# bacpop/ska.rust

Hardware: AMD Instinct MI355X
Metric: genomes/sec ska build+align, 1 000x5 Mbp k=31; bit-exact vs CPU (higher is better)
Workload: dtype u64

## Files before the change

include/skx.h:

```cpp
#ifndef SKX_H
#define SKX_H
#include <stddef.h>
#include <stdint.h>

#ifdef __cplusplus
extern "C" {
#endif

#define SKX_OK        0
#define SKX_EINVAL    1
#define SKX_EIO       2
#define SKX_ENODEV    3
#define SKX_ENOMEM    4
#define SKX_EEMPTY    5
#define SKX_EUNSUP    6
#define SKX_EFORMAT   7

enum { SKX_QUAL_NOFILTER = 0, SKX_QUAL_MIDDLE = 1, SKX_QUAL_STRICT = 2 };
enum { SKX_FILTER_NONE = 0, SKX_FILTER_NO_CONST = 1, SKX_FILTER_NO_AMBIG = 2, SKX_FILTER_NO_AMBIG_OR_CONST = 3 };

typedef struct {
    uint16_t min_count;
    uint8_t  min_qual;
    int32_t  qual_filter;
// ... 96 lines not shown
                               int64_t *constant, uint64_t *rows_used, skx_select_info *info);
int  skx_array_distance_select_prefiltered(skx_array *a, int64_t constant, int filt_ambig, const skx_select_spec *spec, skx_dist_pair **pairs,
                                           uint64_t *n_pairs, skx_select_info *info);
typedef struct { double max_snps, max_mismatches; int32_t band_rows; } skx_mst_spec;
typedef struct { uint64_t bands, band_rows, count_buffer_bytes, candidates, edges, components, rounds; } skx_mst_info;
int  skx_array_distance_mst(skx_array *a, double min_freq, int filt_ambig, const skx_mst_spec *spec, skx_dist_pair **pairs, uint64_t *n_pairs,
                            int64_t *constant, uint64_t *rows_used, skx_mst_info *info);
int  skx_array_distance_mst_prefiltered(skx_array *a, int64_t constant, int filt_ambig, const skx_mst_spec *spec, skx_dist_pair **pairs,
                                        uint64_t *n_pairs, skx_mst_info *info);
int  skx_array_distance_planes(skx_array *a, int filt_ambig, const void **planes, uint64_t *words_per_row, int *n_planes);
int  skx_planes_distance(skx_ctx *ctx, const void *planes, int n_samples, uint64_t words_per_row, int filt_ambig, double constant,
                         int i_lo, int i_hi, skx_dist *out);
void skx_free(void *p);

typedef struct skx_comm skx_comm;
#define SKX_COMM_ID_BYTES 128
int  skx_comm_unique_id(uint8_t id[SKX_COMM_ID_BYTES]);
int  skx_comm_create(skx_ctx *ctx, int rank, int world, const uint8_t id[SKX_COMM_ID_BYTES], skx_comm **out);
int  skx_comm_create_local(skx_ctx *ctx, int rank, int world, const char *dir, skx_comm **out);
void skx_comm_destroy(skx_comm *c);
int  skx_comm_rank(const skx_comm *c);
int  skx_comm_world(const skx_comm *c);
uint64_t skx_comm_bytes_received(const skx_comm *c);
int  skx_comm_transport(const skx_comm *c, int *rccl_ranks, int *rccl_device, int *ctx_device);
int  skx_comm_barrier(skx_comm *c);
int  skx_comm_allgather(skx_comm *c, const void *send, void *recv, uint64_t bytes, int on_device);
int  skx_comm_allreduce_u32(skx_comm *c, uint32_t *buf, uint64_t n, int on_device);
int  skx_comm_gather_root(skx_comm *c, const void *send, const uint64_t *sizes, void *recv);
int  skx_shard_range(uint64_t n_items, int rank, int world, uint64_t *lo, uint64_t *hi);
int  skx_pair_bands(int n_samples, int world, int align, int *lo_hi);
int  skx_keyset_allgather(skx_comm *c, skx_keyset *local, skx_keyset **rows);
int  skx_array_reduce_stats(skx_comm *c, skx_array *a, uint64_t total_samples);
int  skx_array_distance_sharded(skx_comm *c, skx_array *a, int filt_ambig, double constant, skx_dist *out, uint64_t n_out);


int  skx_array_merge(skx_ctx *ctx, skx_array *const *arrays, int n_arrays, skx_array **out);
int  skx_array_delete_samples(skx_array *a, const char *const *names, int n_names);
typedef struct { uint64_t rows_present, removed, silent, sites; } skx_subset_info;
int  skx_array_subset_filtered(skx_array *a, const int *samples, int n_samples, const skx_filter_spec *f,
                               skx_array **out, skx_subset_info *info);
int  skx_array_weed(skx_array *a, skx_keyset *weed, int reverse, uint64_t *removed);
int  skx_keyset_from_fasta(skx_ctx *ctx, const char *path, int k, int rc, skx_keyset **out);
int  skx_cov_histogram(skx_ctx *ctx, const char *fastq_fwd, const char *fastq_rev, int k, int rc, uint32_t *hist);

int  skx_array_map(skx_array *a, const char *reference_fasta, int ambig_mask, int repeat_mask, int format, int threads, char **buf, uint64_t *len);
int  skx_skf_peek_k(const char *path);
skx_ctx *skx_array_ctx(const skx_array *a);
void skx_set_last_error(const char *msg);

typedef struct skx_lo_graph skx_lo_graph;
typedef struct {
    int32_t  k, words_per_node;
    uint64_t n_samples, colour_words;
    uint64_t n_nodes, n_edges, n_entries;
    uint64_t n_colours;
    uint64_t n_kmers;
} skx_lo_info;
int  skx_array_lo_graph(skx_array *a, skx_lo_graph **out);
int  skx_lo_graph_info(const skx_lo_graph *g, skx_lo_info *info);
int  skx_lo_graph_export(const skx_lo_graph *g, uint64_t *nodes, uint64_t *offsets, uint64_t *neighbours, uint64_t *entries, uint64_t *exits);
int  skx_lo_gather(skx_lo_graph *g, const uint64_t *kmers, uint64_t n, uint64_t *colours, uint8_t *found);
void skx_lo_graph_free(skx_lo_graph *g);

typedef struct { uint32_t a, b; double len_a, len_b; } skx_nj_join;
int  skx_dist_nj(skx_ctx *ctx, const skx_dist *d, int n_samples, skx_nj_join *joins);
int  skx_matrix_nj(skx_ctx *ctx, const double *m, int n, skx_nj_join *joins);

typedef struct {
    double  cluster_snps, cluster_mismatches;
    int32_t band_rows;
} skx_banded_spec;
typedef struct { uint64_t bands, band_rows, count_buffer_bytes, edges, clusters; } skx_banded_info;
int  skx_array_distance_banded(skx_array *a, double min_freq, int filt_ambig, const skx_banded_spec *spec,
                               uint32_t *labels, skx_nj_join *joins, int64_t *constant, uint64_t *rows_used, skx_banded_info *info);
int  skx_array_distance_banded_prefiltered(skx_array *a, int64_t constant, int filt_ambig, const skx_banded_spec *spec,
                                           uint32_t *labels, skx_nj_join *joins, skx_banded_info *info);

int  skx_phases_json(char **buf, uint64_t *len, int reset);
void skx_phase_add(const char *name, double seconds);

typedef struct { double hist, scatter, dedupe, key_union, assemble, filter, compact, distance, append_probe, append, pieces_stats, pieces_rows; } skx_timings;
int  skx_ctx_timings(skx_ctx *ctx, skx_timings *t, int reset);
const char *skx_ctx_merge_path(skx_ctx *ctx);

#ifdef __cplusplus
}
#endif
#endif
```

ska.rust_amd/csrc/skx_api.cpp:

```cpp
#include "skx_internal.h"
#include "../../include/skx_host.h"
#include <algorithm>
#include <atomic>
#include <chrono>
#include <cmath>
#include <cstdarg>
#include <cstddef>
#include <cstdio>
#include <cstring>
#include <map>
#include <memory>
#include <mutex>
#include <numeric>
#include <optional>
#include <unordered_map>
#include <thread>
#include <cerrno>
#include <fcntl.h>
#include <sys/mman.h>
#include <sys/stat.h>
#include <unistd.h>

using namespace skx;

// ... 129 lines not shown
}

int skx::check_k(int k)
{
    if (k < 5 || k > 63 || (k & 1) == 0) { set_error("Invalid k-mer length"); return SKX_EINVAL; }
    return SKX_OK;
}

skx::Preallocator::Preallocator(int fd_, off_t base_) : fd(fd_), base(base_)
{
    th = std::thread([this]() {
        constexpr uint64_t STEP = 256ull << 20;
        std::unique_lock<std::mutex> lk(mu);
        for (;;) {
            cv.wait(lk, [this] { return stop || done < target; });
            if (stop && done >= target) return;
            const uint64_t o = done, n = std::min(STEP, target - done);
            lk.unlock();
            if (posix_fallocate(fd, base + (off_t)o, (off_t)n) != 0) failed.store(true, std::memory_order_release);
            lk.lock();
            done = o + n;
            cv.notify_all();
        }
    });
}
skx::Preallocator::~Preallocator() { { std::lock_guard<std::mutex> lk(mu); stop = true; target = done; } cv.notify_all(); if (th.joinable()) th.join(); }
void skx::Preallocator::raise(uint64_t bytes) { { std::lock_guard<std::mutex> lk(mu); if (bytes > target) target = bytes; } cv.notify_all(); }
void skx::Preallocator::finish(uint64_t bytes)
{
    std::unique_lock<std::mutex> lk(mu);
    if (bytes > target) target = bytes;
    cv.notify_all();
    cv.wait(lk, [&] { return done >= bytes; });
}
bool skx::mappable_output_fd(int fd, off_t *pos)
{
    struct stat sb;
    if (fstat(fd, &sb) != 0 || !S_ISREG(sb.st_mode)) return false;
    const int fl = fcntl(fd, F_GETFL);
    if (fl < 0 || (fl & O_APPEND) || (fl & O_ACCMODE) != O_RDWR) return false;
    *pos = lseek(fd, 0, SEEK_CUR);
    return *pos >= 0;
}
extern "C" int skx_ctx_expect_output(skx_ctx *ctx, int fd)
{
    if (!ctx) return SKX_EINVAL;
    off_t pos;
    ctx->expect_fd = (fd >= 0 && mappable_output_fd(fd, &pos)) ? fd : -1;
    return SKX_OK;
}

extern "C" int skx_ctx_create(int device, skx_ctx **out)
{
    return skx_guarded([&]() -> int {
    if (!out) { set_error("null out"); return SKX_EINVAL; }
    int ndev = 0;
    hipError_t e = hipGetDeviceCount(&ndev);
    if (e != hipSuccess || ndev <= 0) { set_error("no HIP device available (%s); the engine has no CPU path", e == hipSuccess ? "count 0" : hipGetErrorString(e)); return SKX_ENODEV; }
    if (device < 0 || device >= ndev) { set_error("device %d out of range (%d devices)", device, ndev); return SKX_EINVAL; }
    SKX_HIP(hipSetDevice(device));
    skx_ctx *c = new skx_ctx();
    c->device = device;
    if (hipStreamCreateWithFlags(&c->stream, hipStreamNonBlocking) != hipSuccess ||
        hipEventCreate(&c->ev[0]) != hipSuccess || hipEventCreate(&c->ev[1]) != hipSuccess || hipEventCreate(&c->ev[2]) != hipSuccess ||
        hipEventCreate(&c->ev[3]) != hipSuccess) {
        delete c; set_error("cannot create HIP stream/events"); return SKX_ENODEV;
    }
    *out = c;
    return SKX_OK;
    });
}
extern "C" void skx_ctx_destroy(skx_ctx *c)
{
    if (!c) return;
    if (c->stream) { (void)hipStreamSynchronize(c->stream); (void)hipStreamDestroy(c->stream); }
    for (auto &e : c->ev) if (e) (void)hipEventDestroy(e);
    skx::dev_trim();
    delete c;
}
extern "C" int skx_ctx_sync(skx_ctx *c) { SKX_HIP(hipSetDevice(c->device)); SKX_HIP(hipStreamSynchronize(c->stream)); return SKX_OK; }
extern "C" void *skx_ctx_stream(skx_ctx *c) { return (void *)c->stream; }
uint64_t skx::next_object_id() { static std::atomic<uint64_t> n{0}; return ++n; }
extern "C" const char *skx_ctx_merge_path(skx_ctx *c) { return c ? c->merge_path.c_str() : ""; }
extern "C" int skx_ctx_timings(skx_ctx *c, skx_timings *t, int reset)
{
    return skx_guarded([&]() -> int {
    if (t) *t = c->tm;
    if (reset) c->tm = skx_timings{};
    return SKX_OK;
    });
}

namespace {
struct KernelTimer {
    skx_ctx *c; double *slot;
    KernelTimer(skx_ctx *c_, double *s) : c(c_), slot(s) { if (c->timing) (void)hipEventRecord(c->ev[2], c->stream); }
    ~KernelTimer()
    {
        if (!c->timing) return;
        (void)hipEventRecord(c->ev[3], c->stream);
        (void)hipEventSynchronize(c->ev[3]);
        float ms = 0; if (hipEventElapsedTime(&ms, c->ev[2], c->ev[3]) == hipSuccess) *slot += ms;
    }
};
int ilog2_ceil(uint64_t x) { int l = 0; while ((1ull << l) < x) l++; return l; }
constexpr uint32_t LDS_TABLE_MAX = 18000;
constexpr uint32_t LDS_SORT_MAX = 6144;
constexpr uint32_t LDS_SORT_MAX_WIDE = 4096;
}

extern "C" void skx_dictset_free(skx_dictset *d) { delete d; }
extern "C" int skx_dictset_nsamples(const skx_dictset *d) { return d->n; }
extern "C" int skx_dictset_key_bits(const skx_dictset *d) { return d->key_bits; }

int skx::reads_words_to_dictset(skx_ctx *ctx, std::vector<DevBuf<uint64_t>> &wl, std::vector<DevBuf<uint64_t>> &wh2, const std::vector<uint64_t> &cnt,
                                int k, int rc, skx_dictset **out)
{
    const int n = (int)wl.size();
    hipStream_t st = ctx->stream;
    const bool wide_r = k > 31;
    const int wpk_r = wide_r ? 2 : 1, kbits = 2 * (k - 1);
    uint64_t maxn = 0;
    for (auto c : cnt) maxn = std::max(maxn, c);
    const uint64_t per = wide_r ? 2500 : 3500, lds_max = wide_r ? LDS_SORT_MAX_WIDE : LDS_SORT_MAX;
    int logB = std::min({ilog2_ceil((maxn + per - 1) / per), kbits, MAX_LOGB});
    if (logB < 0) logB = 0;
    std::unique_ptr<skx_dictset> d(new skx_dictset());
    d->ctx = ctx; d->n = n; d->k = k; d->rc = rc; d->logB = logB; d->hp = make_hash_params(std::min(k, 31)); d->wh = make_wide_hash(k);
    d->key_bits = wide_r ? 128 : 64;
    const uint64_t nreg = (uint64_t)n << logB;
    SKX_TRY(d->raw.alloc(nreg)); SKX_TRY(d->ucnt.alloc(nreg)); SKX_TRY(d->off.alloc(nreg + 1)); SKX_TRY(d->sidx.alloc(nreg * skx::SUBIDX));
    d->sb = std::min(4, kbits - logB);
    SKX_TRY(d->raw.zero(st));
    for (int s = 0; s < n; s++) launch_words_regions(true, wl[s].p, wide_r ? wh2[s].p : nullptr, cnt[s], kbits, logB, (uint64_t)s << logB, d->raw.p, nullptr, nullptr, nullptr, st);
    DevBuf<uint32_t> d_max, cursor; SKX_TRY(d_max.alloc(1)); SKX_TRY(cursor.alloc(nreg)); SKX_TRY(cursor.zero(st));
    launch_scan_u32(d->raw.p, d->off.p, nreg, d_max.p, st);
    uint64_t total = 0; uint32_t max_raw = 0;
    SKX_HIP(hipMemcpyAsync(&total, d->off.p + nreg, 8, hipMemcpyDeviceToHost, st));
    SKX_HIP(hipMemcpyAsync(&max_raw, d_max.p, 4, hipMemcpyDeviceToHost, st));
    SKX_HIP(hipStreamSynchronize(st));
    if (max_raw > lds_max) { if (getenv("SKX_DEBUG")) fprintf(stderr, "[skx] reads: region of %u words, batch left to the sort-based form\n", max_raw); return SKF_NOT_TAKEN; }
    SKX_TRY(d->words.alloc(std::max<uint64_t>(total, 1) * wpk_r));
    for (int s = 0; s < n; s++) {
        launch_words_regions(false, wl[s].p, wide_r ? wh2[s].p : nullptr, cnt[s], kbits, logB, (uint64_t)s << logB, nullptr, d->off.p, cursor.p, d->words.p, st);
        wl[s].release(); wh2[s].release();
    }
    const uint32_t cap = std::max<uint32_t>(512, (uint32_t)std::min<uint64_t>(((uint64_t)max_raw + 255) / 256 * 256, lds_max));
    DevBuf<int> d_flag2; SKX_TRY(d_flag2.alloc(1)); SKX_TRY(d_flag2.zero(st));
    SKX_HIP(hipMemsetAsync(d->sidx.p, 0xFF, nreg * skx::SUBIDX * sizeof(uint16_t), st));
    { StageTimer t(ctx, &ctx->tm.dedupe);
      if (wide_r) launch_dedupe_wide((u128 *)d->words.p, d->off.p, d->raw.p, d->ucnt.p, nreg, cap, kbits - logB, d_flag2.p, d->sidx.p, d->sb, st);
      else launch_dedupe_mb(d->words.p, d->off.p, d->raw.p, d->ucnt.p, nreg, cap, d->hp.bits - logB, d_flag2.p, d->sidx.p, d->sb, st); }
    int overflow = 0;
    std::vector<uint32_t> ucnt(nreg);
    SKX_HIP(hipMemcpyAsync(&overflow, d_flag2.p, 4, hipMemcpyDeviceToHost, st));
    SKX_HIP(hipMemcpyAsync(ucnt.data(), d->ucnt.p, nreg * 4, hipMemcpyDeviceToHost, st));
    SKX_HIP(hipStreamSynchronize(st));
    SKX_HIP(hipGetLastError());
    if (overflow) { if (getenv("SKX_DEBUG")) fprintf(stderr, "[skx] reads: dedupe overflow, batch left to the sort-based form\n"); return SKF_NOT_TAKEN; }
    d->sample_size.assign(n, 0);
    for (int s = 0; s < n; s++) for (uint64_t b = 0; b < (1ull << logB); b++) d->sample_size[s] += ucnt[((uint64_t)s << logB) + b];
    *out = d.release();
    return SKX_OK;

}

// ... 746 lines not shown
        }
        if (rows->wide) launch_gather_keys_wide((const u128 *)rows->stage.p, rows->stride, rows->ncnt.p, rows->roff.p, 1 << rows->logN, (u128 *)a->keys.p, st);
        else launch_gather_keys(rows->stage.p, rows->stride, rows->ncnt.p, rows->roff.p, 1 << rows->logN, a->keys.p, 0, rows->hp, st);
        SKX_HIP(hipMemcpyAsync(a->vcount.p, a->present.p, U * 4, hipMemcpyDeviceToDevice, st));
    }
    int missing = 0;
    SKX_HIP(hipMemcpyAsync(&missing, d_flag.p, 4, hipMemcpyDeviceToHost, st));
    SKX_HIP(hipStreamSynchronize(st));
    SKX_HIP(hipGetLastError());
    if (missing) { set_error("row keyset does not contain every split k-mer of the samples"); return SKX_EINVAL; }
    *out = a.release();
    return SKX_OK;
    });
}

static PiecesRowsArgs pieces_args(skx_array *a)
{
    PiecesRowsArgs pa{};
    const skx_pieces *pc = a->pieces; const skx_keyset *rows = a->lazy_rows;
    pa.pieces = pc->data.p; pa.plen = pc->plen.p; pa.perm = pc->perm.p; pa.nrank = pc->nrank.p; pa.cap = pc->cap; pa.n_samples = (int)a->names.size();
    pa.ncnt = rows->ncnt.p; pa.roff = rows->roff.p;
    return pa;
}
static void launch_assemble_lazy(skx_array *a, const AssembleArgs &aa, hipStream_t st, int mode, uint32_t n_blocks = 0)
{
    if (a->lazy_rows->wide) launch_assemble_wide(aa, st, mode, n_blocks); else launch_assemble(aa, st, mode, n_blocks);
}
static AssembleArgs lazy_args(skx_array *a, int *d_flag)
{
    AssembleArgs aa{};
    skx_keyset *rows = a->lazy_rows;
    aa.d = a->lazy_dict->view(); aa.logN = rows->logN; aa.stage = rows->stage.p; aa.stride = rows->stride; aa.ncnt = rows->ncnt.p; aa.roff = rows->roff.p;
    aa.matrix = nullptr; aa.pitch = 0; aa.col_present = a->present.p; aa.col_unambig = a->unambig.p; aa.col_mask = a->mask.p;
    aa.max_rows = rows->max_rows; aa.missing = d_flag;
    return aa;
}
static int array_make_lazy(skx_ctx *ctx, skx_dictset *d, skx_keyset *rows, const char *const *names, skx_array **out)
{
    std::unique_ptr<skx_array> a(new skx_array());
    a->lazy_dict = d; a->lazy_rows = rows;
    rows->side.release(); rows->perm.release(); rows->g_perm.release(); rows->g_n.release(); rows->g_base.release(); rows->side_of = nullptr;
    hipStream_t st = ctx->stream;
    a->ctx = ctx; a->k = d->k; a->rc = d->rc; a->k_bits = d->key_bits; a->hp = d->hp; a->wh = d->wh; a->version = skx_version();
    for (int i = 0; i < d->n; i++) a->names.emplace_back(names && names[i] ? names[i] : "");
    const uint64_t U = rows->total;
    a->n_rows = a->n_kmers = U; a->pitch = 0; a->engine_order = true; a->stats_ready = false;
    SKX_TRY(a->present.alloc(U)); SKX_TRY(a->unambig.alloc(U)); SKX_TRY(a->mask.alloc(U)); SKX_TRY(a->keys.alloc(U * rows->wpk())); SKX_TRY(a->vcount.alloc(U));
    if (U) {
        if (rows->wide) launch_gather_keys_wide((const u128 *)rows->stage.p, rows->stride, rows->ncnt.p, rows->roff.p, 1 << rows->logN, (u128 *)a->keys.p, st);
        else launch_gather_keys(rows->stage.p, rows->stride, rows->ncnt.p, rows->roff.p, 1 << rows->logN, a->keys.p, 0, rows->hp, st);
    }
    SKX_HIP(hipStreamSynchronize(st));
    *out = a.release();
    return SKX_OK;
}
static int lazy_check_missing(skx_array *a, DevBuf<int> &d_flag)
{
    int missing = 0;
    SKX_HIP(hipMemcpyAsync(&missing, d_flag.p, 4, hipMemcpyDeviceToHost, a->ctx->stream));
    SKX_HIP(hipStreamSynchronize(a->ctx->stream));
    SKX_HIP(hipGetLastError());
    if (missing) { set_error("row keyset does not contain every split k-mer of the samples"); return SKX_EINVAL; }
    return SKX_OK;
}
extern "C" int skx_array_assemble_lazy(skx_ctx *ctx, skx_dictset *d, skx_keyset *rows, const char *const *names, skx_array **out)
{
    return skx_guarded([&]() -> int {
    if (!ctx || !d || !rows || !out) { skx_dictset_free(d); skx_keyset_free(rows); set_error("bad arguments"); return SKX_EINVAL; }
    if (rows->holds_pieces_of(d)) {
        const int r = skx_array_assemble(ctx, d, rows, names, out);
        skx_dictset_free(d); skx_keyset_free(rows);
        return r;
    }
    if (rows->wide != d->wide() || rows->k != d->k || rows->rc != d->rc || rows->logN < 0 || rows->logN < d->logB || d->n > 65535 || knob("eager_array")) {
        const int r = skx_array_assemble(ctx, d, rows, names, out);
        skx_dictset_free(d); skx_keyset_free(rows);
        return r;
    }
    SKX_HIP(hipSetDevice(ctx->device));
    { const int rs = dictset_sort(d); if (rs != SKX_OK) { skx_dictset_free(d); skx_keyset_free(rows); return rs; } }
    return array_make_lazy(ctx, d, rows, names, out);
    });
}
int skx::array_lazy_stats(skx_array *a)
{
    if (!a->lazy() || a->stats_ready) return SKX_OK;
    skx_ctx *ctx = a->ctx; hipStream_t st = ctx->stream;
    SKX_HIP(hipSetDevice(ctx->device));
    DevBuf<int> d_flag; SKX_TRY(d_flag.alloc(1)); SKX_TRY(d_flag.zero(st));
    if (a->n_rows) {
        AssembleArgs aa = lazy_args(a, d_flag.p);
        { StageTimer t(ctx, &ctx->tm.assemble); launch_assemble_lazy(a, aa, st, 1); }
        SKX_HIP(hipMemcpyAsync(a->vcount.p, a->present.p, a->n_rows * 4, hipMemcpyDeviceToDevice, st));
    }
    SKX_TRY(lazy_check_missing(a, d_flag));
    a->stats_ready = true;
    return SKX_OK;
}
int skx::array_materialize(skx_array *a)
{
    if (!a->lazy()) return SKX_OK;
    skx_ctx *ctx = a->ctx; hipStream_t st = ctx->stream;
    SKX_HIP(hipSetDevice(ctx->device));
    const uint64_t U = a->n_rows; const size_t S = a->names.size();
    a->pitch = pitch_for(U);
    SKX_TRY(a->matrix.alloc((uint64_t)S * a->pitch));
    DevBuf<int> d_flag; SKX_TRY(d_flag.alloc(1)); SKX_TRY(d_flag.zero(st));
    if (a->pieces) {
        if (U) {
            PiecesRowsArgs pa = pieces_args(a);
            pa.out = a->matrix.p; pa.pitch = a->pitch;
            { StageTimer t(ctx, &ctx->tm.assemble); launch_pieces_rows(pa, 1u << a->pieces->logQ, st); }
        }
        SKX_HIP(hipStreamSynchronize(st));
        SKX_HIP(hipGetLastError());
        a->drop_lazy();
        return SKX_OK;
    }
    if (U) {
        AssembleArgs aa = lazy_args(a, d_flag.p);
        aa.matrix = a->matrix.p; aa.pitch = a->pitch;
        { StageTimer t(ctx, &ctx->tm.assemble); launch_assemble_lazy(a, aa, st, 0); }
        if (!a->stats_ready) SKX_HIP(hipMemcpyAsync(a->vcount.p, a->present.p, U * 4, hipMemcpyDeviceToDevice, st));
    }
    SKX_TRY(lazy_check_missing(a, d_flag));
    a->stats_ready = true;
    a->drop_lazy();
    return SKX_OK;
}
int skx::array_lazy_window(skx_array *a, uint64_t r0, uint64_t nr, DevBuf<uint8_t> &buf, const uint8_t **win, uint64_t *wpitch)
{
    skx_ctx *ctx = a->ctx; hipStream_t st = ctx->stream;
    skx_keyset *rows = a->lazy_rows;
    if (rows->h_roff.empty()) {
        rows->h_roff.resize((1ull << rows->logN) + 1);
        SKX_HIP(hipMemcpy(rows->h_roff.data(), rows->roff.p, rows->h_roff.size() * 8, hipMemcpyDeviceToHost));
    }
    const auto &ro = rows->h_roff;
    const uint64_t j0 = (uint64_t)(std::upper_bound(ro.begin(), ro.end(), r0) - ro.begin()) - 1;
    const uint64_t j1 = (uint64_t)(std::lower_bound(ro.begin(), ro.end(), r0 + nr) - ro.begin());
    const uint64_t c0 = ro[j0] & ~15ull, span = ro[j1] - c0;
    const uint64_t wp = pitch_for(span);
    const size_t S = a->names.size();
    if (buf.n < S * wp) SKX_TRY(buf.alloc(S * wp));
    if (a->pieces) {
        PiecesRowsArgs pa = pieces_args(a);
        pa.out = buf.p; pa.pitch = wp; pa.j_base = (uint32_t)j0; pa.col_base = c0;
        { StageTimer t(ctx, &ctx->tm.assemble); launch_pieces_rows(pa, (uint32_t)(j1 - j0), st); }
        SKX_HIP(hipGetLastError());
        *win = buf.p + (r0 - c0); *wpitch = wp;
        return SKX_OK;
    }
    DevBuf<int> d_flag; SKX_TRY(d_flag.alloc(1)); SKX_TRY(d_flag.zero(st));
    AssembleArgs aa = lazy_args(a, d_flag.p);
    aa.matrix = buf.p; aa.pitch = wp; aa.j_base = (uint32_t)j0; aa.col_base = c0;
    { StageTimer t(ctx, &ctx->tm.assemble); launch_assemble_lazy(a, aa, st, 0, (uint32_t)(j1 - j0)); }
    SKX_TRY(lazy_check_missing(a, d_flag));
    *win = buf.p + (r0 - c0); *wpitch = wp;
    return SKX_OK;
}

static int append_pass(skx_ctx *ctx, skx_dictset *d, std::unique_ptr<skx_keyset> &ks_out, std::unique_ptr<skx_pieces> &pc_out)
{
    auto not_taken = [&](const char *why) -> int {
        ctx->merge_path = std::string("sorted: ") + why;
        if (getenv("SKX_DEBUG")) fprintf(stderr, "[skx] merge: %s\n", ctx->merge_path.c_str());
        return SKF_NOT_TAKEN;
    };
    if (d->sorted) return not_taken("the dictionaries are sorted (read sets, oversize or repeat-rich samples, SKX_KNOBS=sorted_dicts)");
    if (d->n > 65535 || d->n < 1) return not_taken("more than 65535 samples");
    SKX_HIP(hipSetDevice(ctx->device));
    hipStream_t st = ctx->stream;
    const bool wide = d->wide();
    const int S = d->n, bits = wide ? d->wh.bits : d->hp.bits, logB = d->logB, wpk = wide ? 2 : 1;
    const uint32_t region_cap = d->region_cap;
    const uint32_t max_cap = wide ? APPEND_WIDE_MAX_CAP : APPEND_MAX_CAP, max_slots = wide ? APPEND_WIDE_MAX_SLOTS : APPEND_MAX_SLOTS;
    uint64_t raw_sum = 0, raw_max = 0;
    for (auto v : d->raw_total) { raw_sum += v; raw_max = std::max(raw_max, v); }
    const int min_logQ = std::max(logB, bits - (wide ? 113 : 50));
    if (min_logQ > bits) return not_taken("no row-block split with room for a rank in a table entry");
    auto ranks_for = [&](double mean) -> uint32_t {
        const double c = mean + 6.0 * std::sqrt(mean + 1.0) + 32.0;
        return (uint32_t)std::min<double>(max_cap, std::ceil(c / 128.0) * 128.0);
    };
    auto slots_for = [&](uint32_t cap) -> uint32_t {
        uint32_t n = 256u;
// ... 30 lines not shown
    }
    for (logQ = min_logQ; logQ < bits && u_est / (double)(1ull << logQ) + 6.0 * std::sqrt(u_est / (double)(1ull << logQ) + 1.0) + 32.0 > (double)max_cap; logQ++) { }
    for (int attempt = 0;; attempt++, logQ++) {
        if (logQ > bits || attempt > 3) return not_taken("row blocks kept overflowing (a sample that is one repeat, or far more rows than the probe saw)");
        const uint64_t nsub = 1ull << logQ;
        const double mean = u_est / (double)nsub;
        const uint32_t cap = ranks_for(mean), nslots = slots_for(cap);
        const uint64_t amp = 1ull << (logQ - logB);
        const uint64_t amp_max = region_cap > (wide ? LDS_SORT_MAX_WIDE : LDS_SORT_MAX) ? 32 : 8;
        if (amp > amp_max && (double)raw_sum * (double)amp > 4e8) return not_taken("too many row blocks per region: every region would be read too often");
        if (!pass_ok(logQ, nslots, cap)) return not_taken("no row-block split that fits the LDS");
        std::unique_ptr<skx_keyset> ks(new skx_keyset());
        ks->ctx = ctx; ks->k = d->k; ks->rc = d->rc; ks->logN = logQ; ks->hp = d->hp; ks->wh = d->wh; ks->wide = wide; ks->stride = cap;
        std::unique_ptr<skx_pieces> pc(new skx_pieces());
        pc->cap = cap; pc->logQ = logQ;
        SKX_TRY(ks->stage.alloc(nsub * cap * wpk)); SKX_TRY(ks->ncnt.alloc(nsub));
        if (pc->data.alloc(nsub * (uint64_t)S * (cap / 2)) != SKX_OK) return not_taken("no room for the pieces");
        SKX_TRY(pc->plen.alloc(nsub * (uint64_t)S + 2)); SKX_TRY(pc->perm.alloc(nsub * cap)); SKX_TRY(pc->nrank.alloc(nsub));
        SKX_TRY(d_flag.zero(st));
        aa.logQ = logQ; aa.nslots = nslots; aa.cap = cap;
        aa.rounds = 1; aa.bar = nullptr;
        DevBuf<int> d_bar;
        {
            int cus = 0; (void)hipDeviceGetAttribute(&cus, hipDeviceAttributeMultiprocessorCount, ctx->device);
            uint64_t g = nsub;
            while (g > (uint64_t)std::max(cus, 1) && g % 2 == 0) g /= 2;
            if (g <= (uint64_t)std::max(cus, 1) && nsub % g == 0 && g % (8 * amp) == 0 && logB >= 3) {
                aa.rounds = (uint32_t)(nsub / g);
                SKX_TRY(d_bar.alloc(2ull << logB)); SKX_TRY(d_bar.zero(st)); aa.bar = d_bar.p;
            }
        }
        aa.pieces = pc->data.p; aa.plen = pc->plen.p; aa.perm = pc->perm.p; aa.nrank = pc->nrank.p;
        aa.stage = ks->stage.p; aa.stride = cap; aa.ncnt = ks->ncnt.p;
        { KernelTimer kt(ctx, &ctx->tm.append); if (wide) launch_append_wide(aa, st); else launch_append(aa, region_cap, st); }
        int ov = 0;
        SKX_HIP(hipMemcpyAsync(&ov, d_flag.p, 4, hipMemcpyDeviceToHost, st));
        SKX_HIP(hipStreamSynchronize(st));
        SKX_HIP(hipGetLastError());
        if (getenv("SKX_DEBUG")) fprintf(stderr, "[skx] append%s: logQ=%d (x%llu per region) cap=%u slots=%u rows~%.0f -> %s\n", wide ? " (128-bit keys)" : "", logQ, (unsigned long long)amp, cap, nslots, u_est, ov ? "overflow" : "ok");
        if (ov & 4) return not_taken("the table's bytes are not at LDS address 0");
        if (ov) continue;
        SKX_TRY(keyset_finish(ks.get()));
        ctx->merge_path = wide ? "append128" : "append64";
        ks_out = std::move(ks); pc_out = std::move(pc);
        return SKX_OK;
    }
}
static int array_over_pieces(skx_ctx *ctx, const skx_dictset *d, skx_keyset *ks, skx_pieces *pc_, skx_keyset *g, const char *const *names, skx_array **out)
{
    std::unique_ptr<skx_pieces> pc(pc_);
    hipStream_t st = ctx->stream;
    const int S = d->n, logQ = pc->logQ;
    const uint64_t nsub = 1ull << logQ;
    std::unique_ptr<skx_keyset> blk(new skx_keyset());
    blk->ctx = ctx; blk->k = d->k; blk->rc = d->rc; blk->logN = logQ; blk->hp = d->hp; blk->wh = d->wh; blk->wide = d->wide(); blk->stride = pc->cap;
    uint64_t U;
    if (g) {
        U = g->total;
        pc->perm = std::move(g->g_perm);
        blk->ncnt = std::move(g->g_n);
        SKX_TRY(blk->roff.alloc(nsub + 1));
        SKX_HIP(hipMemcpyAsync(blk->roff.p, g->g_base.p, nsub * 8, hipMemcpyDeviceToDevice, st));
        SKX_HIP(hipMemcpyAsync(blk->roff.p + nsub, &U, 8, hipMemcpyHostToDevice, st));
        SKX_HIP(hipStreamSynchronize(st));
        g->g_base.release();
        blk->total = U; blk->max_rows = g->g_max;
    } else {
        U = ks->total;
        SKX_TRY(blk->ncnt.alloc(nsub)); SKX_TRY(blk->roff.alloc(nsub + 1));
        SKX_HIP(hipMemcpyAsync(blk->ncnt.p, ks->ncnt.p, nsub * 4, hipMemcpyDeviceToDevice, st));
        SKX_HIP(hipMemcpyAsync(blk->roff.p, ks->roff.p, (nsub + 1) * 8, hipMemcpyDeviceToDevice, st));
        blk->total = U; blk->max_rows = ks->max_rows;
    }
    std::unique_ptr<skx_array> a(new skx_array());
    a->ctx = ctx; a->k = d->k; a->rc = d->rc; a->k_bits = d->key_bits; a->hp = d->hp; a->wh = d->wh; a->version = skx_version();
    for (int i = 0; i < S; i++) a->names.emplace_back(names && names[i] ? names[i] : "");
    a->n_rows = a->n_kmers = U; a->pitch = 0; a->engine_order = true; a->stats_ready = true;
    SKX_TRY(a->present.alloc(U)); SKX_TRY(a->unambig.alloc(U)); SKX_TRY(a->mask.alloc(U)); SKX_TRY(a->keys.alloc(U * (d->wide() ? 2 : 1))); SKX_TRY(a->vcount.alloc(U));
    if (U) {
        skx_keyset *src = g ? g : ks;
        if (src->wide) launch_gather_keys_wide((const u128 *)src->stage.p, src->stride, g ? g->ncnt.p : blk->ncnt.p, g ? g->roff.p : blk->roff.p, 1 << src->logN, (u128 *)a->keys.p, st);
        else launch_gather_keys(src->stage.p, src->stride, g ? g->ncnt.p : blk->ncnt.p, g ? g->roff.p : blk->roff.p, 1 << src->logN, a->keys.p, 0, src->hp, st);
        if (g) { SKX_TRY(a->present.zero(st)); SKX_TRY(a->unambig.zero(st)); SKX_TRY(a->mask.zero(st)); SKX_TRY(a->vcount.zero(st)); }
        StageTimer t(ctx, &ctx->tm.assemble);
        KernelTimer kt(ctx, &ctx->tm.pieces_stats);
        launch_pieces_stats(pc->data.p, pc->plen.p, pc->perm.p, pc->nrank.p, blk->ncnt.p, blk->roff.p, pc->cap, S, 1 << logQ, a->present.p, a->unambig.p, a->mask.p, a->vcount.p, st);
    }
    SKX_HIP(hipStreamSynchronize(st));
    SKX_HIP(hipGetLastError());
    a->pieces = pc.release(); a->lazy_rows = blk.release();
    *out = a.release();
    return SKX_OK;
}
static int merge_append(skx_ctx *ctx, skx_dictset *d, const char *const *names, skx_array **out)
{
    std::unique_ptr<skx_keyset> ks; std::unique_ptr<skx_pieces> pc;
    const int r = append_pass(ctx, d, ks, pc);
    if (r != SKX_OK) return r;
    return array_over_pieces(ctx, d, ks.get(), pc.release(), nullptr, names, out);
}

extern "C" int skx_merge(skx_ctx *ctx, skx_dictset *d, const char *const *names, skx_array **out)
{
    return skx_guarded([&]() -> int {
    if (!ctx || !d || !out) { set_error("bad arguments"); return SKX_EINVAL; }
    { const int ra = merge_append(ctx, d, names, out); if (ra != SKF_NOT_TAKEN) return ra; }
    skx_keyset *ks = nullptr;
    SKX_TRY(keyset_union_dict(ctx, d, &ks, true));
    int r = skx_array_assemble(ctx, d, ks, names, out);
    skx_keyset_free(ks);
    return r;
    });
}

struct SampleNeed { uint64_t resident = 0, transient = 0; };
static SampleNeed sample_device_bytes(const char *f1, const char *f2, bool wide, unsigned min_count)
{
    uint64_t bytes = 0; bool reads = false;
    for (const char *f : sample_files(f1, f2)) {
        const FileProbe p = probe_file(f);
        if (!p.found) continue;
        const bool gz = p.n_head >= 1 && p.head[0] == 0x1f;
        reads |= gz || (p.n_head >= 1 && p.head[0] == '@');
        bytes += p.size * (gz ? 5u : 1u);
    }
    SampleNeed n;
    if (reads) {
        const uint64_t bases = bytes / 2;
        n.resident = bytes + bases / std::max(1u, min_count) * (wide ? 20u : 12u) + (8u << 20);
        n.transient = bases * (wide ? 56u : 28u);
    } else
        n.resident = bytes * (wide ? 44u : 24u) + (8u << 20);
    return n;
}
static uint64_t cached_device_bytes()
{
    const int dev = current_device();
    std::lock_guard<std::mutex> lk(g_cache.mu);
    uint64_t n = 0;
    auto it = g_cache.free_blocks.find(dev);
    if (it != g_cache.free_blocks.end()) for (auto &kv : it->second) n += kv.first;
    return n;
}
static uint64_t build_budget_bytes(skx_ctx *ctx)
{
    if (const char *e = getenv("SKX_BUILD_BATCH_MB")) return (uint64_t)std::max(1.0, atof(e)) << 20;
    size_t fr = 0, tot = 0;
    if (hipSetDevice(ctx->device) != hipSuccess || hipMemGetInfo(&fr, &tot) != hipSuccess) return ~0ull;
    return (uint64_t)(fr + cached_device_bytes()) / 10 * 6;
}
static int build_range(skx_ctx *ctx, const char *const *names, const char *const *file1, const char *const *file2, int lo, int hi,
                       int k, int rc, const skx_qual *q, int threads, double proportion_reads, std::vector<skx_array *> &parts)
{
    skx_dictset *d = nullptr;
    skx_array *a = nullptr;
    int r = skx_dictset_build_files(ctx, file1 + lo, file2 ? file2 + lo : nullptr, hi - lo, k, rc, q, threads, proportion_reads, &d);
    if (r == SKX_OK) {
        const auto t0 = std::chrono::steady_clock::now();
        int ra = merge_append(ctx, d, names + lo, &a);
        if (ra != SKF_NOT_TAKEN) r = ra;
        else if (!knob("eager_array")) {
            skx_keyset *ks = nullptr;
            r = skx_keyset_union(ctx, d, &ks);
            if (r == SKX_OK) r = array_make_lazy(ctx, d, ks, names + lo, &a); else skx_dictset_free(d);
            d = nullptr;
        } else
// ... 168 lines not shown
    std::vector<uint8_t> rm(variants ? U * S : 0);
    std::vector<uint32_t> pres(U);
    if (U) {
        if (variants) {
            DevBuf<uint8_t> d_rm; SKX_TRY(d_rm.alloc(U * S));
            launch_transpose(a->matrix.p, a->pitch, S, U, d_rm.p, S, st);
            SKX_HIP(hipMemcpyAsync(rm.data(), d_rm.p, U * S, hipMemcpyDeviceToHost, st));
            SKX_HIP(hipStreamSynchronize(st));
        }
        SKX_HIP(hipMemcpyAsync(pres.data(), a->vcount.p, U * 4, hipMemcpyDeviceToHost, st));
        SKX_HIP(hipStreamSynchronize(st));
    }
    std::vector<uint64_t> idx(U); std::iota(idx.begin(), idx.end(), 0);
    const bool in_step = K == U;
    if (in_step) std::sort(idx.begin(), idx.end(), [&](uint64_t x, uint64_t y) { return hk[x].hi != hk[y].hi ? hk[x].hi < hk[y].hi : hk[x].lo < hk[y].lo; });
    if (keys) { if (in_step) for (uint64_t i = 0; i < K; i++) keys[i] = hk[idx[i]]; else std::copy(hk.begin(), hk.end(), keys); }
    if (variants) for (uint64_t i = 0; i < U; i++) memcpy(variants + i * S, rm.data() + idx[i] * S, S);
    if (counts) for (uint64_t i = 0; i < U; i++) counts[i] = pres[idx[i]];
    return SKX_OK;
    });
}

extern "C" int skx_array_sample_kmers(skx_array *a, int64_t *out)
{
    return skx_guarded([&]() -> int {
    skx_ctx *ctx = a->ctx; hipStream_t st = ctx->stream;
    SKX_HIP(hipSetDevice(ctx->device));
    const size_t S = a->names.size();
    if (a->pieces) {
        skx_pieces *pc = a->pieces;
        if (pc->sample_cells.size() != S) {
            DevBuf<unsigned long long> d; SKX_TRY(d.alloc(S)); SKX_TRY(d.zero(st));
            launch_pieces_cells(pc->data.p, pc->plen.p, pc->cap, (int)S, 1 << pc->logQ, d.p, st);
            std::vector<unsigned long long> h(S);
            SKX_HIP(hipMemcpyAsync(h.data(), d.p, S * 8, hipMemcpyDeviceToHost, st));
            SKX_HIP(hipStreamSynchronize(st));
            pc->sample_cells.assign(h.begin(), h.end());
        }
        for (size_t i = 0; i < S; i++) out[i] = (int64_t)pc->sample_cells[i];
        return SKX_OK;
    }
    if (a->lazy()) { for (size_t i = 0; i < S; i++) out[i] = (int64_t)a->lazy_dict->sample_size[i]; return SKX_OK; }
    DevBuf<unsigned long long> d; SKX_TRY(d.alloc(S)); SKX_TRY(d.zero(st));
    launch_row_nonmissing(a->matrix.p, a->pitch, (int)S, a->n_rows, d.p, st);
    std::vector<unsigned long long> h(S);
    SKX_HIP(hipMemcpyAsync(h.data(), d.p, S * 8, hipMemcpyDeviceToHost, st));
    SKX_HIP(hipStreamSynchronize(st));
    for (size_t i = 0; i < S; i++) out[i] = (int64_t)h[i];
    return SKX_OK;
    });
}

extern "C" int skx_array_pieces_info(skx_array *a, uint64_t *piece_bytes, uint64_t *row_blocks, uint32_t *ranks_per_block)
{
    return skx_guarded([&]() -> int {
    if (!a) { set_error("bad arguments"); return SKX_EINVAL; }
    if (piece_bytes) *piece_bytes = 0;
    if (row_blocks) *row_blocks = 0;
    if (ranks_per_block) *ranks_per_block = 0;
    const skx_pieces *pc = a->pieces;
    if (!pc) return SKX_OK;
    skx_ctx *ctx = a->ctx; hipStream_t st = ctx->stream;
    SKX_HIP(hipSetDevice(ctx->device));
    const uint64_t n = ((uint64_t)1 << pc->logQ) * a->names.size();
    std::vector<uint16_t> h(n);
    SKX_HIP(hipMemcpyAsync(h.data(), pc->plen.p, n * 2, hipMemcpyDeviceToHost, st));
    SKX_HIP(hipStreamSynchronize(st));
    uint64_t b = 0;
    for (uint16_t v : h) b += ((uint64_t)v + 31) / 32 * 16;
    if (piece_bytes) *piece_bytes = b;
    if (row_blocks) *row_blocks = (uint64_t)1 << pc->logQ;
    if (ranks_per_block) *ranks_per_block = pc->cap;
    return SKX_OK;
    });
}

static int array_compact(skx_array *a, DevBuf<uint8_t> &keep, DevBuf<uint64_t> &pos, uint64_t kept, int mask_ambig, bool vcount_from_unambig,
                         bool keys_follow)
{
    skx_ctx *ctx = a->ctx; hipStream_t st = ctx->stream;
    const uint64_t U = a->n_rows; const size_t S = a->names.size();
    const bool filter_ambig_as_missing = vcount_from_unambig;
    if (kept == U && !mask_ambig) {
        if (filter_ambig_as_missing && U) SKX_HIP(hipMemcpyAsync(a->vcount.p, a->unambig.p, U * 4, hipMemcpyDeviceToDevice, st));
        SKX_HIP(hipStreamSynchronize(st));
        return SKX_OK;
    }
    {
        StageTimer t(ctx, &ctx->tm.compact);
        const uint64_t np = pitch_for(kept);
        DevBuf<uint8_t> nm; DevBuf<uint32_t> p2, u2, m2, v2;
        SKX_TRY(nm.alloc((uint64_t)S * np)); SKX_TRY(p2.alloc(kept)); SKX_TRY(u2.alloc(kept)); SKX_TRY(m2.alloc(kept)); SKX_TRY(v2.alloc(kept));
        if (a->pieces) {
            PiecesRowsArgs pa = pieces_args(a);
            pa.out = nm.p; pa.pitch = np; pa.keep = keep.p; pa.kpos = pos.p; pa.mask_ambig = mask_ambig;
            KernelTimer kt(ctx, &ctx->tm.pieces_rows);
            launch_pieces_rows(pa, 1u << a->pieces->logQ, st);
        } else if (a->lazy()) {
            DevBuf<int> d_flag; SKX_TRY(d_flag.alloc(1)); SKX_TRY(d_flag.zero(st));
            AssembleArgs aa = lazy_args(a, d_flag.p);
            aa.matrix = nm.p; aa.pitch = np; aa.keep = keep.p; aa.kpos = pos.p; aa.mask_ambig = mask_ambig;
            { StageTimer t2(ctx, &ctx->tm.assemble); launch_assemble_lazy(a, aa, st, 2); }
            SKX_TRY(lazy_check_missing(a, d_flag));
        } else
            launch_compact_matrix(a->matrix.p, a->pitch, nm.p, np, (int)S, U, keep.p, pos.p, mask_ambig, st);
        launch_compact_u32(a->present.p, p2.p, U, keep.p, pos.p, st);
        launch_compact_u32(a->unambig.p, u2.p, U, keep.p, pos.p, st);
        launch_compact_u32(a->mask.p, m2.p, U, keep.p, pos.p, st);
        launch_compact_u32(filter_ambig_as_missing ? a->unambig.p : a->vcount.p, v2.p, U, keep.p, pos.p, st);
        if (mask_ambig) launch_mask_ambig_stats(m2.p, kept, st);
        if (a->n_kmers == U && keys_follow) {
            if (a->k <= 31) {
                DevBuf<uint64_t> k2; SKX_TRY(k2.alloc(kept));
                launch_compact_u64(a->keys.p, k2.p, U, keep.p, pos.p, st);
                a->keys = std::move(k2);
            } else if (a->host_keys.empty()) {
                DevBuf<uint64_t> k2; SKX_TRY(k2.alloc(kept * 2));
                launch_compact_u128(a->keys.p, k2.p, U, keep.p, pos.p, st);
                a->keys = std::move(k2);
            } else {
                std::vector<uint8_t> hkeep(U);
                SKX_HIP(hipMemcpyAsync(hkeep.data(), keep.p, U, hipMemcpyDeviceToHost, st));
                SKX_HIP(hipStreamSynchronize(st));
                std::vector<skx_key> nk; nk.reserve(kept);
                for (uint64_t i = 0; i < U; i++) if (hkeep[i] == 1) nk.push_back(a->host_keys[i]);
                a->host_keys.swap(nk);
            }
            a->n_kmers = kept;
        }
        SKX_HIP(hipStreamSynchronize(st));
        a->matrix = std::move(nm); a->present = std::move(p2); a->unambig = std::move(u2); a->mask = std::move(m2); a->vcount = std::move(v2);
        a->pitch = np; a->n_rows = kept;
        a->drop_lazy();
    }
    return SKX_OK;
}

extern "C" int skx_array_filter(skx_array *a, uint64_t min_count, int filter_ambig_as_missing, int filter_type, int mask_ambig,
                                int ignore_const_gaps, int update_kmers, int32_t *removed)
{
    return skx_guarded([&]() -> int {
    skx_ctx *ctx = a->ctx; hipStream_t st = ctx->stream;
    SKX_HIP(hipSetDevice(ctx->device));
    const uint64_t U = a->n_rows; const size_t S = a->names.size();
    SKX_TRY(array_lazy_stats(a));
    DevBuf<uint8_t> keep; DevBuf<uint64_t> pos;
    SKX_TRY(keep.alloc(U)); SKX_TRY(pos.alloc(U + 1));
    uint64_t kept = 0, silent = 0;
    {
        StageTimer t(ctx, &ctx->tm.filter);
        FilterArgs fa{a->vcount.p, a->present.p, a->unambig.p, a->mask.p, U, (uint32_t)(a->total_samples ? a->total_samples : S), min_count, filter_ambig_as_missing, filter_type, ignore_const_gaps, keep.p};
        launch_filter_flags(fa, st);
        DevBuf<uint32_t> sc_sums; DevBuf<uint64_t> sc_offs;
        SKX_TRY(sc_sums.alloc(scan_u8_blocks(U))); SKX_TRY(sc_offs.alloc(scan_u8_blocks(U) + 1));
        launch_scan_u8(keep.p, pos.p, U, sc_sums.p, sc_offs.p, st);
        SKX_HIP(hipMemcpyAsync(&kept, pos.p + U, 8, hipMemcpyDeviceToHost, st));
        if (filter_ambig_as_missing) {
            DevBuf<unsigned long long> d_sil; SKX_TRY(d_sil.alloc(1)); SKX_TRY(d_sil.zero(st));
            launch_count_u8(keep.p, U, 2, d_sil.p, st);
            unsigned long long s2 = 0;
            SKX_HIP(hipMemcpyAsync(&s2, d_sil.p, 8, hipMemcpyDeviceToHost, st));
            SKX_HIP(hipStreamSynchronize(st));
            silent = s2;
        }
        SKX_HIP(hipStreamSynchronize(st));
    }
    SKX_TRY(array_compact(a, keep, pos, kept, mask_ambig, filter_ambig_as_missing != 0, update_kmers || filter_ambig_as_missing));
    SKX_HIP(hipGetLastError());
    if (removed) *removed = (int32_t)(U - kept - silent);
    return SKX_OK;
    });
}


static int array_keep_rows(skx_array *a, DevBuf<uint8_t> &keep, uint64_t *removed)
{
    hipStream_t st = a->ctx->stream;
    const uint64_t U = a->n_rows;
    DevBuf<uint64_t> pos; SKX_TRY(pos.alloc(U + 1));
    uint64_t kept = 0;
    DevBuf<uint32_t> sc_sums; DevBuf<uint64_t> sc_offs;
    SKX_TRY(sc_sums.alloc(scan_u8_blocks(U))); SKX_TRY(sc_offs.alloc(scan_u8_blocks(U) + 1));
    launch_scan_u8(keep.p, pos.p, U, sc_sums.p, sc_offs.p, st);
    SKX_HIP(hipMemcpyAsync(&kept, pos.p + U, 8, hipMemcpyDeviceToHost, st));
    SKX_HIP(hipStreamSynchronize(st));
    SKX_TRY(array_compact(a, keep, pos, kept, 0, false, true));
    SKX_HIP(hipGetLastError());
    if (removed) *removed = U - kept;
    return SKX_OK;
}

extern "C" skx_ctx *skx_array_ctx(const skx_array *a) { return a->ctx; }
extern "C" void skx_set_last_error(const char *msg) { set_error("%s", msg ? msg : ""); }

extern "C" int skx_keyset_from_fasta(skx_ctx *ctx, const char *path, int k, int rc, skx_keyset **out)
{
    return skx_guarded([&]() -> int {
    if (!ctx || !path || !out) { set_error("bad arguments"); return SKX_EINVAL; }
    SKX_TRY(check_k(k));
    HostStream hs;
    SKX_TRY(read_sample_stream(path, nullptr, 0.0, hs));
    if (hs.is_fastq) { set_error("Cannot create reference from FASTQ files"); return SKX_EINVAL; }
    skx_stream ss; ss.seq = hs.seq.data(); ss.qual = nullptr; ss.len = hs.seq.size();
    skx_dictset *d = nullptr;
    int r = skx_dictset_build(ctx, &ss, 1, 0, k, rc, nullptr, &d);
    if (r == SKX_EEMPTY) set_error("%s has no valid sequence", path);
    if (r != SKX_OK) return r;
    r = skx_keyset_union(ctx, d, out);
    skx_dictset_free(d);
    return r;
    });
}

extern "C" int skx_array_merge(skx_ctx *ctx, skx_array *const *in, int n, skx_array **out)
{
    return skx_guarded([&]() -> int {
    if (!ctx || !in || n <= 0 || !out) { set_error("bad arguments"); return SKX_EINVAL; }
    SKX_HIP(hipSetDevice(ctx->device));
    hipStream_t st = ctx->stream;
    uint64_t tot = 0; size_t S = 0;
    for (int i = 0; i < n; i++) SKX_TRY(array_materialize(in[i]));
    for (int i = 0; i < n; i++) {
        if (in[i]->k != in[0]->k) { set_error("K-mer lengths do not match: %d %d", in[i]->k, in[0]->k); return SKX_EINVAL; }
        if (in[i]->rc != in[0]->rc) { set_error("Strand use inconsistent"); return SKX_EINVAL; }
        if (in[i]->n_kmers != in[i]->n_rows || in[i]->keys_absent) { set_error("split k-mers and variants are out of step (filtered without update_kmers)"); return SKX_EINVAL; }
        tot += in[i]->n_rows; S += in[i]->names.size();
    }
    if (S > 65535) { set_error("more than 65535 samples per device array"); return SKX_EUNSUP; }
// ... 306 lines not shown
```

ska.rust_amd/csrc/skx_append.hip:

```cpp
#include "skx_device.h"
#include <cstdlib>
#include <type_traits>

namespace skx {

typedef uint32_t u32x4 __attribute__((ext_vector_type(4)));
typedef const u32x4 __attribute__((address_space(1))) *g4_t;

#ifdef SKX_AP_PROF
__device__ unsigned long long g_ap_prof[16];
#define AP_PROF_START unsigned long long tprof = __builtin_readcyclecounter(), tacc[12] = {0, 0, 0, 0, 0, 0, 0, 0, 0, 0, 0, 0}
#define AP_PROF(i) do { const unsigned long long t_ = __builtin_readcyclecounter(); tacc[(i)] += t_ - tprof; tprof = t_; } while (0)
#define AP_PROF_FLUSH() do { for (int i_ = 0; i_ < 12; i_++) if (tacc[i_] && (i_ >= 6 || (threadIdx.x & 63) == 0)) atomicAdd(&g_ap_prof[i_], tacc[i_]); } while (0)
extern "C" void skx_debug_phase_prof(unsigned long long *out, int reset)
{
    unsigned long long h[16];
    (void)hipDeviceSynchronize();
    (void)hipMemcpyFromSymbol(h, HIP_SYMBOL(g_ap_prof), sizeof(h));
    for (int i = 0; i < 16; i++) out[i] = h[i];
    if (reset) { for (auto &x : h) x = 0; (void)hipMemcpyToSymbol(HIP_SYMBOL(g_ap_prof), h, sizeof(h)); }
}
#else
#define AP_PROF_START do { } while (0)
#define AP_PROF(i) do { } while (0)
// ... 376 lines not shown
                        __syncthreads();
                        if (tid == 0) {
                            int *ctr = a.bar + (1 << a.logB) + region;
                            const int want = (int)A * (it / (AP_RESYNC > 0 ? AP_RESYNC : 1));
                            atomicAdd(ctr, 1);
                            for (int spin = 0; spin < (1 << 16) && __hip_atomic_load(ctr, __ATOMIC_RELAXED, __HIP_MEMORY_SCOPE_AGENT) < want; spin++) __builtin_amdgcn_s_sleep(4);
                        }
                        __syncthreads();
                    }
                }
            } else c++;
        }
        asm volatile("s_waitcnt vmcnt(0)" ::: "memory");
    }
    AP_PROF_FLUSH();
    __syncthreads();
    const uint32_t nr = s_ctl[CTL_NROWS];
    if (s_ctl[CTL_FAIL]) { if (tid == 0) atomicOr(a.overflow, (int)s_ctl[CTL_FAIL]); __syncthreads(); continue; }
    uint32_t *s_tmp = s_ctl + CTL_TMP;
    if (COUNT_ONLY) {
        uint32_t c = 0;
        for (uint32_t i = tid; i < total_slots; i += AP_THREADS) c += s_tab[i] != 0ull;
        uint32_t tot; (void)ap_block_excl(c, s_tmp, &tot);
        if (tid == 0) { atomicAdd(&a.probe[0], (unsigned long long)tot); atomicMax(&a.probe[1], (unsigned long long)tot); }
        continue;
    }
    uint16_t *s_perm = reinterpret_cast<uint16_t *>(s_q);
    for (uint32_t i = tid; i < cap; i += AP_THREADS) s_perm[i] = 0xFFFFu;
    __syncthreads();
    const uint32_t per = (total_slots + AP_THREADS - 1) / AP_THREADS;
    const uint32_t lo = tid * per, hi = lo + per < total_slots ? lo + per : total_slots;
    uint32_t c = 0;
    for (uint32_t i = lo; i < hi; i++) c += s_tab[i] != 0ull;
    uint32_t total;
    uint32_t pos = ap_block_excl(c, s_tmp, &total);
    uint64_t *slab = a.stage + j * (uint64_t)a.stride;
    for (uint32_t i = lo; i < hi; i++) {
        const unsigned long long e = s_tab[i];
        if (!e) continue;
        uint32_t gl = 0, lr = 0;
        for (int64_t t = (int64_t)i - 1; t >= 0; t--) { const unsigned long long o = s_tab[t]; if (!o) break; gl += o > e; }
        for (uint32_t t = i + 1; t < total_slots; t++) { const unsigned long long o = s_tab[t]; if (!o) break; lr += o < e; }
        const uint32_t idx = pos - gl + lr, rank = ((uint32_t)e & AP_RANK_MASK) - 1u;
        pos++;
        if (idx < a.stride && rank < cap) {
            uint64_t hl;
            if (HI) hl = ((uint64_t)(uint32_t)(e >> 32) << lowb) | (uint64_t)((uint32_t)e >> AP_RANK_BITS);
            else hl = rem == 0 ? 0ull : (uint64_t)((uint32_t)(e >> 32) >> (32 - rem));
            slab[idx] = ((((uint64_t)j << rem) | hl) << 4) | 1ull;
            s_perm[rank] = (uint16_t)idx;
        }
    }
    __syncthreads();
    uint16_t *pj = a.perm + j * (uint64_t)cap;
    for (uint32_t i = tid; i < cap; i += AP_THREADS) pj[i] = s_perm[i];
    if (tid == 0) { a.ncnt[j] = total; a.nrank[j] = nr < cap ? nr : cap; if (total > a.stride) atomicOr(a.overflow, 1); }
    __syncthreads();
    }
}

template <bool COUNT_ONLY>
static void launch_append_t(const AppendArgs &a, unsigned blocks, hipStream_t st)
{
    const size_t lds = append_lds_bytes(a.nslots, a.cap, COUNT_ONLY);
    const bool hi = a.bits - a.logQ >= 32;
    if (hi) {
        (void)hipFuncSetAttribute((const void *)append_kernel<COUNT_ONLY, true>, hipFuncAttributeMaxDynamicSharedMemorySize, (int)lds);
        hipLaunchKernelGGL((append_kernel<COUNT_ONLY, true>), dim3(blocks), dim3(AP_THREADS), lds, st, a);
    } else {
        (void)hipFuncSetAttribute((const void *)append_kernel<COUNT_ONLY, false>, hipFuncAttributeMaxDynamicSharedMemorySize, (int)lds);
        hipLaunchKernelGGL((append_kernel<COUNT_ONLY, false>), dim3(blocks), dim3(AP_THREADS), lds, st, a);
    }
}
bool append_ok(int bits, int logB, int logQ, uint32_t region_cap, uint32_t nslots, uint32_t cap)
{
    const int rem = bits - logQ;
    (void)region_cap;
    return logQ >= logB && rem >= 0 && rem <= 50 && cap % 128u == 0 && cap >= 128u && cap <= APPEND_MAX_CAP && nslots >= cap && (nslots & (nslots - 1u)) == 0u &&
           append_lds_bytes(nslots, cap, false) <= 160u * 1024u - 256u;
}
void launch_append(const AppendArgs &a, uint32_t region_cap, hipStream_t st) { (void)region_cap; launch_append_t<false>(a, (1u << a.logQ) / a.rounds, st); }
void launch_append_probe(const AppendArgs &a, uint32_t region_cap, unsigned blocks, hipStream_t st) { (void)region_cap; launch_append_t<true>(a, blocks, st); }

__global__ __launch_bounds__(256) void pieces_stats_kernel(const uint8_t *pieces, const uint16_t *plen, const uint16_t *perm, const uint32_t *nrank, const uint32_t *ncnt,
                                                           const uint64_t *roff, uint32_t cap, int S, uint32_t *o_present, uint32_t *o_unambig, uint32_t *o_mask,
                                                           uint32_t *o_vcount, int force_direct, uint32_t stage)
{
    constexpr int W = 4;
    extern __shared__ __attribute__((aligned(16))) uint16_t s_stage[];
    const uint32_t PS_STAGE = stage;
    uint16_t *const s_pr = s_stage, *const s_un = s_stage + stage, *const s_mk = s_stage + 2 * (size_t)stage;
    const uint64_t j = blockIdx.x;
    const uint32_t nr = nrank[j], nrows = ncnt[j];
    const uint64_t r0 = roff[j];
    const uint32_t d = blockIdx.y * 256u + threadIdx.x;
    if (blockIdx.y * 256u * 8u * W >= nr && !(blockIdx.y == 0 && nrows)) return;
    const bool staged = gridDim.y == 1 && nrows <= PS_STAGE && !force_direct;
    if (staged) {
        for (uint32_t p = threadIdx.x; p < nrows; p += 256) { s_pr[p] = 0; s_un[p] = 0; s_mk[p] = 0; }
        __syncthreads();
    }
    const int lane = threadIdx.x & 63, wv = threadIdx.x >> 6;
    const uint16_t *pl = plen + j * (uint64_t)S;
    const uint4 *col = reinterpret_cast<const uint4 *>(pieces + j * (uint64_t)S * (cap / 2)) + d;
    const uint32_t step = cap / 32;
    const bool mine = d * 32u < nr;
    uint32_t pN[W], aN[W];
    uint32_t pE[W], pO[W], aE[W], aO[W], uni[W];
    uint32_t PE0[W], PE1[W], PO0[W], PO1[W], AE0[W], AE1[W], AO0[W], AO1[W];
#pragma unroll
    for (int w = 0; w < W; w++) { pN[w] = aN[w] = 0; pE[w] = pO[w] = aE[w] = aO[w] = uni[w] = 0; PE0[w] = PE1[w] = PO0[w] = PO1[w] = AE0[w] = AE1[w] = AO0[w] = AO1[w] = 0; }
    auto nibfold = [&]() {
#pragma unroll
        for (int w = 0; w < W; w++) {
            pE[w] += pN[w] & 0x0F0F0F0Fu; pO[w] += (pN[w] >> 4) & 0x0F0F0F0Fu; aE[w] += aN[w] & 0x0F0F0F0Fu; aO[w] += (aN[w] >> 4) & 0x0F0F0F0Fu;
            pN[w] = aN[w] = 0;
        }
    };
    auto fold = [&]() {
        nibfold();
#pragma unroll
        for (int w = 0; w < W; w++) {
            PE0[w] += pE[w] & 0x00FF00FFu; PE1[w] += (pE[w] >> 8) & 0x00FF00FFu; PO0[w] += pO[w] & 0x00FF00FFu; PO1[w] += (pO[w] >> 8) & 0x00FF00FFu;
            AE0[w] += aE[w] & 0x00FF00FFu; AE1[w] += (aE[w] >> 8) & 0x00FF00FFu; AO0[w] += aO[w] & 0x00FF00FFu; AO1[w] += (aO[w] >> 8) & 0x00FF00FFu;
            pE[w] = pO[w] = aE[w] = aO[w] = 0;
        }
    };
    auto take = [&](int w, uint32_t x) {
        uint32_t t = x | (x >> 1); t |= t >> 2;
        const uint32_t nz = t & 0x11111111u;
        const uint32_t y = x & (x - nz);
        uint32_t u = y | (y >> 1); u |= u >> 2;
        const uint32_t am = u & 0x11111111u;
        pN[w] += nz; aN[w] += am;
        uni[w] |= x;
    };
    for (int s0 = 0, since = 0, nib = 0; s0 < S; s0 += 64) {
        const uint32_t plv = s0 + lane < S ? (uint32_t)pl[s0 + lane] : 0u;
        const int n = S - s0 < 64 ? S - s0 : 64;
#pragma unroll 1
        for (int i0 = 0; i0 < n; i0 += 4) {
            if (nib == 12) { nibfold(); nib = 0; }
            nib += 4;
            uint4 x[4];
#pragma unroll
            for (int u = 0; u < 4; u++) {
                const uint32_t l = (uint32_t)__builtin_amdgcn_readlane((int)plv, (i0 + u) & 63);
                x[u] = make_uint4(0u, 0u, 0u, 0u);
                if (mine && i0 + u < n && d * 32u < l) x[u] = col[(uint64_t)(s0 + i0 + u) * step];
            }
#pragma unroll
            for (int u = 0; u < 4; u++) { take(0, x[u].x); take(1, x[u].y); take(2, x[u].z); take(3, x[u].w); }
        }
        since += 64;
        if (since >= 192) { fold(); since = 0; nib = 0; }
    }
    fold();
    const uint16_t *pj = perm + j * (uint64_t)cap;
    if (mine) {
#pragma unroll
        for (int w = 0; w < W; w++) {
            uint32_t pres[8], amb[8];
            pres[0] = PE0[w] & 0xFFFFu; pres[4] = PE0[w] >> 16; pres[2] = PE1[w] & 0xFFFFu; pres[6] = PE1[w] >> 16;
            pres[1] = PO0[w] & 0xFFFFu; pres[5] = PO0[w] >> 16; pres[3] = PO1[w] & 0xFFFFu; pres[7] = PO1[w] >> 16;
            amb[0] = AE0[w] & 0xFFFFu; amb[4] = AE0[w] >> 16; amb[2] = AE1[w] & 0xFFFFu; amb[6] = AE1[w] >> 16;
            amb[1] = AO0[w] & 0xFFFFu; amb[5] = AO0[w] >> 16; amb[3] = AO1[w] & 0xFFFFu; amb[7] = AO1[w] >> 16;
            const uint4 pv = *reinterpret_cast<const uint4 *>(pj + d * 32u + (uint32_t)w * 8u);
            const uint32_t pw[4] = {pv.x, pv.y, pv.z, pv.w};
#pragma unroll
            for (int i = 0; i < 8; i++) {
                const uint32_t r = d * 32u + (uint32_t)w * 8u + i;
                if (r >= nr) break;
                const uint32_t p = (pw[i >> 1] >> (16 * (i & 1))) & 0xFFFFu;
                if (p >= nrows) continue;
                const uint32_t u = (uni[w] >> (4 * i)) & 15u;
                const uint32_t mk = ((u & 1u) << 1) | ((u & 2u) << 1) | ((u & 4u) << 2) | ((u & 8u) << 5);
                if (staged) { s_pr[p] = (uint16_t)pres[i]; s_un[p] = (uint16_t)(pres[i] - amb[i]); s_mk[p] = (uint16_t)mk; }
                else {
                    o_vcount[r0 + p] = pres[i];
                    __hip_atomic_store(&o_present[r0 + p], pres[i], __ATOMIC_RELAXED, __HIP_MEMORY_SCOPE_AGENT);
                    __hip_atomic_store(&o_unambig[r0 + p], pres[i] - amb[i], __ATOMIC_RELAXED, __HIP_MEMORY_SCOPE_AGENT);
                    o_mask[r0 + p] = mk;
                }
            }
        }
    }
    if (!staged) __threadfence();
    __syncthreads();
    const uint32_t rk0 = blockIdx.y * 256u * 8u * W, rk1 = rk0 + 256u * 8u * W < nr ? rk0 + 256u * 8u * W : nr;
    for (uint32_t rb = rk0 + (uint32_t)wv * 64u; rb < rk1; rb += 256u) {
        const uint32_t rr = rb + (uint32_t)lane;
        uint32_t pp = 0xFFFFu; bool hit = false;
        if (rr < rk1) {
            pp = pj[rr];
            if (pp < nrows) {
                if (staged) hit = s_un[pp] != s_pr[pp];
                else hit = __hip_atomic_load(&o_unambig[r0 + pp], __ATOMIC_RELAXED, __HIP_MEMORY_SCOPE_AGENT) != __hip_atomic_load(&o_present[r0 + pp], __ATOMIC_RELAXED, __HIP_MEMORY_SCOPE_AGENT);
            }
        }
        unsigned long long todo = __ballot(hit);
        while (todo) {
            const int src = __builtin_ctzll(todo);
            todo &= todo - 1;
            const uint32_t r = rb + (uint32_t)src, prow = (uint32_t)__shfl((int)pp, src, 64);
            uint32_t m = 0;
            for (int t = lane; t < S; t += 64) {
                if ((uint32_t)pl[t] <= r) continue;
                const uint32_t x = *(reinterpret_cast<const uint32_t *>(pieces + (j * (uint64_t)S + t) * (cap / 2)) + (r >> 3));
                const uint32_t nib = (x >> ((r & 7u) * 4u)) & 15u;
                if (nib) m |= 1u << nib;
            }
#pragma unroll
            for (int dd = 32; dd >= 1; dd >>= 1) m |= __shfl_xor(m, dd, 64);
            if (lane == 0) { if (staged) s_mk[prow] = (uint16_t)m; else o_mask[r0 + prow] = m; }
        }
    }
    if (!staged) return;
    __syncthreads();
    for (uint32_t p = threadIdx.x; p < nrows; p += 256) {
        const uint32_t pr = s_pr[p];
        o_present[r0 + p] = pr; o_vcount[r0 + p] = pr;
        o_unambig[r0 + p] = s_un[p]; o_mask[r0 + p] = s_mk[p];
    }
}
void launch_pieces_stats(const uint8_t *pieces, const uint16_t *plen, const uint16_t *perm, const uint32_t *nrank, const uint32_t *ncnt, const uint64_t *roff, uint32_t cap,
                         int n_samples, int n_blocks, uint32_t *present, uint32_t *unambig, uint32_t *mask, uint32_t *vcount, hipStream_t st)
{
    if (n_blocks <= 0) return;
    const unsigned gy = (cap / 32 + 255u) / 256u;
    static const int direct = knob("stats_direct") ? 1 : 0;
    const uint32_t stage = (cap + 63u) / 64u * 64u;
    hipLaunchKernelGGL(pieces_stats_kernel, dim3((unsigned)n_blocks, gy), dim3(256), (size_t)stage * 6, st, pieces, plen, perm, nrank, ncnt, roff, cap, n_samples, present, unambig, mask, vcount,
                       direct, stage);
}
__global__ __launch_bounds__(256) void pieces_cells_kernel(const uint8_t *pieces, const uint16_t *plen, uint32_t cap, int S, unsigned long long *out)
{
    const uint64_t j = blockIdx.x;
    const int lane = threadIdx.x & 63;
    for (int s = blockIdx.y * 4 + (threadIdx.x >> 6); s < S; s += gridDim.y * 4) {
        const uint32_t pl = plen[j * (uint64_t)S + s];
        const uint32_t *src = reinterpret_cast<const uint32_t *>(pieces + (j * (uint64_t)S + s) * (cap / 2));
        uint32_t c = 0;
        for (uint32_t i = lane; i < (pl + 7u) / 8u; i += 64) { const uint32_t x = src[i]; uint32_t t = x | (x >> 1); t |= t >> 2; c += (uint32_t)__popc(t & 0x11111111u); }
#pragma unroll
        for (int dd = 32; dd >= 1; dd >>= 1) c += __shfl_xor(c, dd, 64);
        if (lane == 0 && c) atomicAdd(&out[s], (unsigned long long)c);
    }
}
void launch_pieces_cells(const uint8_t *pieces, const uint16_t *plen, uint32_t cap, int n_samples, int n_blocks, unsigned long long *out, hipStream_t st)
{
    if (n_blocks <= 0 || n_samples <= 0) return;
    unsigned gy = (unsigned)((n_samples + 3) / 4); if (gy > 16) gy = 16;
    hipLaunchKernelGGL(pieces_cells_kernel, dim3((unsigned)n_blocks, gy), dim3(256), 0, st, pieces, plen, cap, n_samples, out);
}
__global__ __launch_bounds__(256) void region_totals_kernel(const uint32_t *raw, int logB, unsigned long long *out)
{
    __shared__ unsigned long long s_sum[256];
    const uint64_t B = 1ull << logB;
    unsigned long long t = 0;
    for (uint64_t b = threadIdx.x; b < B; b += 256) t += raw[(uint64_t)blockIdx.x * B + b];
    s_sum[threadIdx.x] = t;
    __syncthreads();
    for (int d = 128; d >= 1; d >>= 1) { if ((int)threadIdx.x < d) s_sum[threadIdx.x] += s_sum[threadIdx.x + d]; __syncthreads(); }
    if (threadIdx.x == 0) out[blockIdx.x] = s_sum[0];
}
void launch_region_totals(const uint32_t *raw, int n_samples, int logB, unsigned long long *out, hipStream_t st)
{
    if (n_samples > 0) hipLaunchKernelGGL(region_totals_kernel, dim3((unsigned)n_samples), dim3(256), 0, st, raw, logB, out);
}

constexpr int PR_WAVES = 8;
__device__ static inline uint32_t ap_iupac4(uint32_t m)
{
    const uint32_t idx = m & 0x07070707u;
    const uint32_t lo = __builtin_amdgcn_perm(0x48595754u, 0x4D43412Du, idx);
    const uint32_t hi = __builtin_amdgcn_perm(0x4E42444Bu, 0x56535247u, idx);
    const uint32_t sel = ((m >> 3) & 0x01010101u) * 0xFFu;
    return (hi & sel) | (lo & ~sel);
}
template <bool KEPT>
__global__ __launch_bounds__(64 * PR_WAVES) void pieces_rows_kernel(PiecesRowsArgs a)
{
    extern __shared__ __attribute__((aligned(16))) unsigned char s_raw[];
    const uint32_t cap = a.cap;
    uint16_t *s_src = reinterpret_cast<uint16_t *>(s_raw);
    uint32_t *s_piece = reinterpret_cast<uint32_t *>(s_raw + (((size_t)cap + 16) * 2 + 15) / 16 * 16);
    const uint64_t j = (uint64_t)blockIdx.x + a.j_base;
    const uint32_t n = a.ncnt[j];
    if (n == 0) return;
    const uint64_t r0 = a.roff[j];
    const uint64_t k0 = KEPT ? a.kpos[r0] : 0;
    const uint32_t nout = KEPT ? (uint32_t)(a.kpos[r0 + n] - k0) : n;
    if (nout == 0) return;
    const int tid = threadIdx.x, lane = tid & 63, wv = tid >> 6;
    const uint64_t ocol = KEPT ? k0 : r0 - a.col_base;
    const uint32_t shift = (uint32_t)(ocol & 3u);
    const uint32_t ndw = (nout + shift + 3u) / 4u;
    const uint16_t *pj = a.perm + j * (uint64_t)cap;
    const uint32_t nr = a.nrank[j];
    const int S = a.n_samples;
    const int s_lo = blockIdx.y * a.samples_per_wg, s_hi = s_lo + a.samples_per_wg < S ? s_lo + a.samples_per_wg : S;
    uint32_t *pc = s_piece + (size_t)wv * (cap / 8 + 4);
    const unsigned char *pcb = reinterpret_cast<const unsigned char *>(pc);
    const uint32_t nrw = (nr + 7u) / 8u;
    if (lane < 4) pc[cap / 8 + lane] = 0u;
    for (uint32_t t0 = 0; t0 < nout + shift; t0 += cap) {
        for (uint32_t i = tid; i < cap + 16u; i += blockDim.x) s_src[i] = (uint16_t)cap;
        __syncthreads();
        for (uint32_t r = tid; r < nr; r += blockDim.x) {
            const uint32_t p = pj[r];
            if (p == 0xFFFFu || p >= n) continue;
            uint32_t sc;
            if (!KEPT) sc = shift + p;
            else if (a.keep[r0 + p] == 1) sc = shift + (uint32_t)(a.kpos[r0 + p] - k0);
            else continue;
            if (sc >= t0 && sc < t0 + cap) s_src[sc - t0] = (uint16_t)r;
        }
        __syncthreads();
        const uint32_t v_lo = t0 / 4u, v_hi = (t0 + cap) / 4u < ndw ? (t0 + cap) / 4u : ndw;
        for (int s = s_lo + wv; s < s_hi; s += PR_WAVES) {
            const uint32_t pl = a.plen[j * (uint64_t)S + s];
            const uint32_t plw = (pl + 7u) / 8u;
            const uint32_t *src = reinterpret_cast<const uint32_t *>(a.pieces + (j * (uint64_t)S + s) * (cap / 2));
            {
                const uint4 *src4 = reinterpret_cast<const uint4 *>(src);
                uint4 *pc4 = reinterpret_cast<uint4 *>(pc);
                for (uint32_t i = lane; i < (nrw + 3u) / 4u; i += 64) {
                    uint4 x = 4u * i < plw ? src4[i] : make_uint4(0u, 0u, 0u, 0u);
                    if (4u * i + 1u >= plw) x.y = 0u;
                    if (4u * i + 2u >= plw) x.z = 0u;
                    if (4u * i + 3u >= plw) x.w = 0u;
                    pc4[i] = x;
                }
            }
            __builtin_amdgcn_wave_barrier();
            unsigned char *dst = a.out + (uint64_t)s * a.pitch + (ocol - shift);
            for (uint32_t v = v_lo + lane; v < v_hi; v += 64) {
                const uint2 rr = *reinterpret_cast<const uint2 *>(s_src + 4u * (v - v_lo));
                const uint32_t ra = rr.x & 0xFFFFu, rb = rr.x >> 16, rc = rr.y & 0xFFFFu, rd = rr.y >> 16;
                const uint32_t na = ((uint32_t)pcb[ra >> 1] >> ((ra & 1u) * 4u)) & 15u, nb = ((uint32_t)pcb[rb >> 1] >> ((rb & 1u) * 4u)) & 15u;
                const uint32_t nc = ((uint32_t)pcb[rc >> 1] >> ((rc & 1u) * 4u)) & 15u, nd = ((uint32_t)pcb[rd >> 1] >> ((rd & 1u) * 4u)) & 15u;
                uint32_t m = na | (nb << 8) | (nc << 16) | (nd << 24);
                uint32_t word = ap_iupac4(m);
                if (a.mask_ambig) {
                    const uint32_t y = m & (m - ((m | (m >> 1) | (m >> 2) | (m >> 3)) & 0x01010101u));
                    const uint32_t amb = ((y | (y >> 1) | (y >> 2) | (y >> 3)) & 0x01010101u) * 0xFFu;
                    word = (word & ~amb) | (0x4E4E4E4Eu & amb);
                }
                const bool head = v == 0 && shift != 0, tail = v == ndw - 1 && ((nout + shift) & 3u) != 0;
                if (!head && !tail) *reinterpret_cast<uint32_t *>(dst + 4u * v) = word;
                else {
#pragma unroll
                    for (int b = 0; b < 4; b++) { const int c = (int)(4u * v + b) - (int)shift; if (c >= 0 && (uint32_t)c < nout) dst[4u * v + b] = (unsigned char)(word >> (8 * b)); }
                }
            }
            __builtin_amdgcn_wave_barrier();
        }
        __syncthreads();
    }
}
void launch_pieces_rows(const PiecesRowsArgs &a, uint32_t n_blocks, hipStream_t st)
{
    if (!n_blocks || a.n_samples <= 0) return;
    PiecesRowsArgs b = a;
    int spw = a.n_samples;
    while (spw > PR_WAVES * 4 && (uint64_t)n_blocks * ((a.n_samples + spw - 1) / spw) < 8192) spw = (spw + 1) / 2;
    b.samples_per_wg = spw;
    const unsigned gy = (unsigned)((a.n_samples + spw - 1) / spw);
    const size_t lds = (((size_t)a.cap + 16) * 2 + 15) / 16 * 16 + (size_t)PR_WAVES * (a.cap / 8 + 4) * 4;
    if (a.keep) {
        (void)hipFuncSetAttribute((const void *)pieces_rows_kernel<true>, hipFuncAttributeMaxDynamicSharedMemorySize, (int)lds);
        hipLaunchKernelGGL(pieces_rows_kernel<true>, dim3(n_blocks, gy), dim3(64 * PR_WAVES), lds, st, b);
    } else {
        (void)hipFuncSetAttribute((const void *)pieces_rows_kernel<false>, hipFuncAttributeMaxDynamicSharedMemorySize, (int)lds);
        hipLaunchKernelGGL(pieces_rows_kernel<false>, dim3(n_blocks, gy), dim3(64 * PR_WAVES), lds, st, b);
    }
}

}

#include "skx_append_wide.inc"
```

ska.rust_amd/csrc/skx_device.h:

```cpp
#pragma once
#include <hip/hip_runtime.h>
#include <stdint.h>

namespace skx {

long knob(const char *name, long absent = 0);
int extract_tile_bases(int logB);
constexpr int MAX_LOGB = 13;
constexpr uint64_t EMPTY64 = ~0ull;

struct HashParams {
    int bits;
    int hb;
    uint32_t hmask;
    uint32_t c[4];
};
HashParams make_hash_params(int k);
__host__ __device__ inline uint32_t hround(uint32_t v, uint32_t c, int hb) { return (v * c) >> (32 - hb); }
__host__ __device__ inline void hmix_halves(uint32_t &L, uint32_t &R, const HashParams &p)
{
    L ^= hround(R, p.c[0], p.hb); R ^= hround(L, p.c[1], p.hb);
}
__host__ __device__ inline uint64_t hmix(uint64_t x, const HashParams &p)
{
// ... 44 lines not shown
    uint32_t *hist;
    const uint64_t *off;
    uint64_t *words;
    uint32_t capacity;
    int *overflow;
};

void launch_hist(const ExtractArgs &a, hipStream_t st);
void launch_scatter(const ExtractArgs &a, hipStream_t st);

void launch_fill_offsets(uint64_t *off, uint64_t n, uint32_t capacity, hipStream_t st);
void launch_scan_u32(const uint32_t *in, uint64_t *out, uint64_t n, uint32_t *max_out, hipStream_t st);

constexpr int SUBIDX = 16;
void launch_dedupe(uint64_t *words, const uint64_t *off, const uint32_t *raw, uint32_t *ucnt, uint64_t n_regions,
                   uint32_t table_slots, int rem_bits, int *overflow, uint32_t min_n, uint16_t *sidx, int sb, hipStream_t st);

uint32_t dedupe_spill_grid();
void launch_dedupe_mb(uint64_t *words, const uint64_t *off, const uint32_t *raw, uint32_t *ucnt, uint64_t n_regions,
                      uint32_t cap, int rem_bits, int *overflow, uint16_t *sidx, int sb, hipStream_t st,
                      uint32_t typical = 0, uint32_t *big_list = nullptr, uint32_t big_from = 0);

struct DictView {
    const uint64_t *words; const uint64_t *off; const uint32_t *ucnt;
    int n_samples, logB, bits;
    const uint16_t *sidx = nullptr; int sb = 0;
};

void launch_union(const DictView &d, int logN, uint64_t *stage, uint32_t stride, uint32_t *ncnt,
                  uint32_t table_slots, int *overflow, hipStream_t st);
void launch_union_probe(const DictView &d, int logP, int probe, uint32_t *cnt, uint32_t table_slots, int *overflow,
                        hipStream_t st);

struct AssembleArgs {
    DictView d;
    int logN;
    const uint64_t *stage;
    uint32_t stride;
    const uint32_t *ncnt;
    const uint64_t *roff;
    uint8_t *matrix;
    uint64_t pitch;
    uint32_t *col_present;
    uint32_t *col_unambig;
    uint32_t *col_mask;
    uint32_t max_rows;
    int *missing;
    uint32_t j_base = 0;
    uint64_t col_base = 0;
    const uint8_t *keep = nullptr; const uint64_t *kpos = nullptr;
    int mask_ambig = 0;
};
void launch_assemble(const AssembleArgs &a, hipStream_t st, int mode = 0, uint32_t n_blocks = 0);
bool union_side_ok(const DictView &d, int logN, uint32_t stride);
void launch_union_side(const DictView &d, int logN, uint64_t *stage, uint32_t stride, uint32_t *ncnt, uint32_t table_slots, int *overflow,
                       uint16_t *side, uint16_t *perm, hipStream_t st);
void launch_assemble_side(const AssembleArgs &a, const uint16_t *side, const uint16_t *perm, hipStream_t st, bool wide = false);
void launch_compose_perm(const uint64_t *l_stage, uint32_t l_stride, const uint32_t *l_ncnt, const uint16_t *l_perm, int l_logN, const uint64_t *g_stage,
                         uint32_t g_stride, const uint32_t *g_ncnt, const uint64_t *g_roff, int g_logN, int bits, uint16_t *g_perm, uint32_t *g_n,
                         uint64_t *g_base, uint32_t *g_max, int *bad, hipStream_t st);
void launch_union_side_wide(const DictView &d, int logN, u128 *stage, uint32_t stride, uint32_t *ncnt, uint32_t table_slots, int *overflow,
                            uint16_t *side, uint16_t *perm, hipStream_t st);

constexpr uint32_t APPEND_MAX_CAP = 6016, APPEND_MAX_SLOTS = 8192;
struct AppendArgs {
    const uint64_t *words; const uint64_t *off; const uint32_t *raw;
    int n_samples, logB, bits, logQ;
    uint32_t nslots, cap;
    uint8_t *pieces; uint16_t *plen; uint16_t *perm; uint32_t *nrank;
    uint64_t *stage; uint32_t stride; uint32_t *ncnt;
    unsigned long long *probe;
    int *overflow;
    uint32_t rounds = 1;
    int *bar = nullptr;
};
bool append_ok(int bits, int logB, int logQ, uint32_t region_cap, uint32_t nslots, uint32_t cap);
void launch_append(const AppendArgs &a, uint32_t region_cap, hipStream_t st);
void launch_append_probe(const AppendArgs &a, uint32_t region_cap, unsigned blocks, hipStream_t st);
constexpr uint32_t APPEND_WIDE_MAX_CAP = 3072, APPEND_WIDE_MAX_SLOTS = 4096;
bool append_wide_ok(int bits, int logB, int logQ, uint32_t nslots, uint32_t cap);
void launch_append_wide(const AppendArgs &a, hipStream_t st);
void launch_append_wide_probe(const AppendArgs &a, unsigned blocks, hipStream_t st);
void launch_pieces_stats(const uint8_t *pieces, const uint16_t *plen, const uint16_t *perm, const uint32_t *nrank, const uint32_t *ncnt, const uint64_t *roff, uint32_t cap,
                         int n_samples, int n_blocks, uint32_t *present, uint32_t *unambig, uint32_t *mask, uint32_t *vcount, hipStream_t st);
void launch_pieces_cells(const uint8_t *pieces, const uint16_t *plen, uint32_t cap, int n_samples, int n_blocks, unsigned long long *out, hipStream_t st);
void launch_region_totals(const uint32_t *raw, int n_samples, int logB, unsigned long long *out, hipStream_t st);
struct PiecesRowsArgs {
    const uint8_t *pieces; const uint16_t *plen; const uint16_t *perm; const uint32_t *nrank; uint32_t cap; int n_samples;
    const uint32_t *ncnt; const uint64_t *roff;
    uint8_t *out; uint64_t pitch;
    uint32_t j_base = 0; uint64_t col_base = 0;
    const uint8_t *keep = nullptr; const uint64_t *kpos = nullptr;
    int mask_ambig = 0;
    int samples_per_wg = 0;
};
void launch_pieces_rows(const PiecesRowsArgs &a, uint32_t n_blocks, hipStream_t st);

void launch_gather_keys(const uint64_t *stage, uint32_t stride, const uint32_t *ncnt, const uint64_t *roff, int n_sub,
                        uint64_t *out, int unhash, HashParams hp, hipStream_t st);
void launch_hash_keys(const uint64_t *keys, uint64_t *words, uint64_t n, HashParams hp, hipStream_t st);
void launch_keys_cbor(const uint64_t *words, uint64_t n, HashParams hp, uint8_t *out, int *short_key, hipStream_t st);
void launch_unhash_dict(const uint64_t *words, uint64_t n, uint64_t *keys, uint8_t *bases, HashParams hp, hipStream_t st);

void launch_col_stats(const uint8_t *matrix, uint64_t pitch, int n_samples, uint64_t n_cols, uint32_t *present,
                      uint32_t *unambig, uint32_t *mask, int *bad_byte, hipStream_t st);
struct FilterArgs {
    const uint32_t *vcount, *present, *unambig, *mask; uint64_t n_cols; uint32_t n_samples;
    uint64_t min_count; int ambig_as_missing, filter_type, ignore_const_gaps;
    uint8_t *keep;
    int two_stage = 0;
};
void launch_filter_flags(const FilterArgs &a, hipStream_t st);
void launch_row_stats_rm(const uint8_t *cells, uint64_t S, uint64_t nr, uint32_t *present, uint32_t *unambig, uint32_t *mask, int *bad_byte, hipStream_t st);
void launch_compact_rm(const uint8_t *cells, uint64_t S, uint64_t nr, const uint8_t *keep, const uint64_t *pos, uint8_t *out, uint64_t pitch,
                       uint64_t col0, int mask_ambig, hipStream_t st);
uint64_t scan_u8_blocks(uint64_t n);
void launch_scan_u8(const uint8_t *flags, uint64_t *pos, uint64_t n, uint32_t *sums, uint64_t *offs, hipStream_t st);
void launch_compact_matrix(const uint8_t *in, uint64_t in_pitch, uint8_t *out, uint64_t out_pitch, int n_samples,
                           uint64_t n_cols, const uint8_t *keep, const uint64_t *pos, int mask_ambig, hipStream_t st, const int *order = nullptr);
void launch_subset_verdicts(const uint8_t *matrix, uint64_t pitch, const int *order, int n, uint64_t n_cols, uint64_t min_count, int ambig_as_missing,
                            int filter_type, int ignore_const_gaps, uint8_t *keep, unsigned long long *counts, int *bad_byte, hipStream_t st);
void launch_compact_u32(const uint32_t *in, uint32_t *out, uint64_t n, const uint8_t *keep, const uint64_t *pos, hipStream_t st);
void launch_compact_u64(const uint64_t *in, uint64_t *out, uint64_t n, const uint8_t *keep, const uint64_t *pos, hipStream_t st);
void launch_compact_u128(const uint64_t *in, uint64_t *out, uint64_t n, const uint8_t *keep, const uint64_t *pos, hipStream_t st);
void launch_mask_ambig_stats(uint32_t *mask, uint64_t n, hipStream_t st);
void launch_count_u8(const uint8_t *v, uint64_t n, uint8_t value, unsigned long long *out, hipStream_t st);
void launch_differ_u32(const uint32_t *a, const uint32_t *b, uint64_t n, int *flag, hipStream_t st);
void launch_transpose(const uint8_t *in, uint64_t in_pitch, uint64_t rows, uint64_t cols, uint8_t *out, uint64_t out_pitch,
                      hipStream_t st);
struct SnapChunk { uint64_t src_off, uoff; uint32_t src_len, ulen, crc, compressed; };
constexpr uint32_t SKF_SLOT = 8 + 65536;
int launch_skf_decode_cells(int device, const uint8_t *src, const SnapChunk *chunks, uint32_t n_chunks, uint64_t upos, uint64_t uend,
                            uint8_t *scratch , uint8_t *cells, uint64_t base_cell, int *status, hipStream_t st);
int launch_skf_encode_cells(int device, const uint8_t *cells, uint64_t base_cell, uint64_t upos, uint64_t uoff0, uint32_t n_chunks,
                            uint8_t *slots, uint32_t *sizes, hipStream_t st);
void launch_skf_gather(const uint8_t *slots, const uint32_t *sizes, const uint64_t *off, uint32_t n_chunks, uint8_t *dense, hipStream_t st);
void launch_row_nonmissing(const uint8_t *matrix, uint64_t pitch, int n_samples, uint64_t n_cols, unsigned long long *out,
                           hipStream_t st);

void launch_build_planes(const uint8_t *matrix, uint64_t pitch, int n_samples, uint64_t n_cols, uint64_t *planes, uint64_t wpr, int filt,
                         hipStream_t st, const int *order = nullptr);
void launch_keep_bits(const uint8_t *keep, const uint64_t *pos, uint64_t n, uint64_t *keep_bits, uint64_t *gpos, hipStream_t st);
void launch_split_keep(const uint8_t *keep, const uint32_t *col_mask, uint64_t n, uint8_t *clean, uint8_t *dirty, hipStream_t st, int mode = 0);
void launch_split_keep_from_dirty(uint8_t *dirty, uint64_t n, uint8_t *clean, hipStream_t st);
void launch_build_planes_keep(const uint8_t *matrix, uint64_t pitch, int n_samples, uint64_t n_cols, const uint64_t *keep_bits, const uint64_t *gpos,
                              uint64_t *planes, uint64_t wpr, int filt, hipStream_t st, uint32_t *first_group, uint64_t kept, const int *order = nullptr);
constexpr int DIST_NCOUNT = 16;
int launch_pair_counts(const uint64_t *planes, int n_samples, uint64_t words_per_row, int filt_ambig,
                       unsigned long long *out, hipStream_t st, int i_lo = 0, int i_hi = 0);

void launch_hist_wide(const ExtractArgs &a, hipStream_t st);
void launch_scatter_wide(const ExtractArgs &a, hipStream_t st);
int extract_tile_bases_wide();
void launch_dedupe_wide(u128 *words, const uint64_t *off, const uint32_t *raw, uint32_t *ucnt, uint64_t n_regions, uint32_t cap,
                        int rem_bits, int *overflow, uint16_t *sidx, int sb, hipStream_t st);
void launch_union_wide(const DictView &d, int logN, u128 *stage, uint32_t stride, uint32_t *ncnt, uint32_t table_slots, int *overflow,
                       hipStream_t st);
void launch_union_probe_wide(const DictView &d, int logP, int probe, uint32_t *cnt, uint32_t table_slots, int *overflow, hipStream_t st);
void launch_assemble_wide(const AssembleArgs &a, hipStream_t st, int mode = 0, uint32_t n_blocks = 0);
void launch_gather_keys_wide(const u128 *stage, uint32_t stride, const uint32_t *ncnt, const uint64_t *roff, int n_sub, u128 *out,
                             hipStream_t st);

uint64_t fasta_parse_tiles(uint64_t len);
#ifdef __HIPCC__
__device__ static inline void planes_bytes16(const uint64_t *groups, uint64_t t, uint64_t len, uint32_t sw[4], uint32_t qw[4])
{
    const uint64_t p0 = t * 16;
    const uint64_t *g = groups + (t >> 2) * 5;
    const int sh = (int)(t & 3) * 16;
    const uint32_t lo = (uint32_t)(g[0] >> sh) & 0xFFFFu, hi = (uint32_t)(g[1] >> sh) & 0xFFFFu, bad = (uint32_t)(g[2] >> sh) & 0xFFFFu,
                   nl = (uint32_t)(g[3] >> sh) & 0xFFFFu, qb = (uint32_t)(g[4] >> sh) & 0xFFFFu;
#pragma unroll
    for (int i = 0; i < 4; i++) {
        uint32_t x = 0, y = 0;
#pragma unroll
        for (int b = 0; b < 4; b++) {
            const int j = 4 * i + b;
            const uint32_t code = ((lo >> j) & 1u) | (((hi >> j) & 1u) << 1);
            const bool isnl = ((nl >> j) & 1u) || p0 + (uint64_t)j >= len;
            const uint32_t c = isnl ? 10u : ((bad >> j) & 1u) ? 78u : (0x47544341u >> (8 * code)) & 0xFFu;
            const uint32_t q = isnl ? 10u : ((qb >> j) & 1u) ? 33u : 32u;
            x |= c << (8 * b); y |= q << (8 * b);
        }
        sw[i] = x; qw[i] = y;
    }
}
#endif
void launch_expand_planes(const uint64_t *groups, uint64_t len, uint8_t *seq, uint8_t *qual, hipStream_t st);
void launch_fasta_parse(const uint8_t *const *raw, const uint64_t *rawlen, uint8_t *const *out, uint64_t *outlen, const uint32_t *tile_file,
                        const uint64_t *tile_base, uint64_t n_tiles, void *summary, uint64_t *tile_off, uint8_t *tile_kind, int n, hipStream_t st);

void launch_lookup_rows(const uint64_t *words, uint64_t n, const uint64_t *sorted, uint64_t m, uint32_t *idx, hipStream_t st);
void launch_lookup_rows_wide(const u128 *words, uint64_t n, const u128 *sorted, uint64_t m, uint32_t *idx, hipStream_t st);
void launch_hash_keys_wide(const u128 *keys, u128 *words, uint64_t n, const WideHash &wh, hipStream_t st);
void launch_map_lookup_wide(const uint64_t *wlo, const uint64_t *whi, const uint8_t *flag, const uint8_t *seq, uint64_t len, int h, const u128 *sorted,
                            const uint32_t *perm, uint64_t U, uint32_t *row, uint8_t *is_rc, hipStream_t st);
void launch_member_flags(const uint32_t *idx, uint64_t n, int reverse, uint8_t *keep, hipStream_t st);
void launch_scatter_rows(const uint8_t *src, uint64_t src_pitch, int n_samples, uint8_t *dst, uint64_t dst_pitch, const uint32_t *idx,
                         uint64_t n, hipStream_t st);
void launch_nonzero_flags(const uint32_t *v, uint64_t n, uint8_t *keep, hipStream_t st);

struct MapWriteArgs {
    const uint8_t *mv; uint64_t mpitch, M;
    const uint32_t *m_pos, *m_chrom;
    const uint64_t *mlo, *mhi;
// ... 16 lines not shown
```

ska.rust_amd/csrc/skx_device2.inc:

```
namespace skx {

__device__ static inline uint32_t set_code(uint32_t b)
{
    switch (b) {
    case '-': return 0;
    case 'A': return 1;  case 'C': return 2;  case 'M': return 3;  case 'T': return 4;
    case 'W': return 5;  case 'Y': return 6;  case 'H': return 7;  case 'G': return 8;
    case 'R': return 9;  case 'S': return 10; case 'V': return 11; case 'K': return 12;
    case 'D': return 13; case 'B': return 14; case 'N': return 15;
    default: return 0xFF;
    }
}

__global__ __launch_bounds__(256) void col_stats_kernel(const uint8_t *matrix, uint64_t pitch, int n_samples, uint64_t n_cols,
                                                        uint32_t *present, uint32_t *unambig, uint32_t *mask, int *bad_byte)
{
    const uint64_t c0 = ((uint64_t)blockIdx.x * blockDim.x + threadIdx.x) * 4;
    if (c0 >= n_cols) return;
    uint32_t p[4] = {0, 0, 0, 0}, u[4] = {0, 0, 0, 0}, m[4] = {0, 0, 0, 0};
    int bad = 0;
    for (int s = 0; s < n_samples; s++) {
        const uint32_t x = *reinterpret_cast<const uint32_t *>(matrix + (uint64_t)s * pitch + c0);
#pragma unroll
        for (int i = 0; i < 4; i++) {
// ... 113 lines not shown
        (void)hipFuncSetAttribute((const void *)compact_matrix_kernel<true>, hipFuncAttributeMaxDynamicSharedMemorySize, (int)lds);
        hipLaunchKernelGGL(compact_matrix_kernel<true>, grid, dim3(256), lds, st, in, in_pitch, out, out_pitch, n_samples, n_cols, keep, pos, mask_ambig, order);
        return;
    }
    (void)hipFuncSetAttribute((const void *)compact_matrix_kernel<false>, hipFuncAttributeMaxDynamicSharedMemorySize, (int)lds);
    hipLaunchKernelGGL(compact_matrix_kernel<false>, grid, dim3(256), lds, st, in, in_pitch, out, out_pitch, n_samples, n_cols, keep, pos, mask_ambig, order);
}

__global__ __launch_bounds__(256) void subset_verdict_kernel(const uint8_t *matrix, uint64_t pitch, const int *order, int n, uint64_t n_cols, uint64_t min_count,
                                                             int ambig_as_missing, int filter_type, int ignore_const_gaps, uint8_t *keep,
                                                             unsigned long long *counts, int *bad_byte)
{
    __shared__ uint8_t s_lut[256];
    __shared__ uint32_t s_cnt[4][3];
    s_lut[threadIdx.x] = (uint8_t)set_code(threadIdx.x);
    __syncthreads();
    const uint64_t c0 = ((uint64_t)blockIdx.x * 256 + threadIdx.x) * 16;
    uint32_t n_absent = 0, n_silent = 0, n_removed = 0;
    if (c0 < n_cols) {
        uint32_t pu[16], m[16];
#pragma unroll
        for (int i = 0; i < 16; i++) { pu[i] = 0; m[i] = 0; }
        uint32_t bad = 0;
        typedef uint32_t u32x4 __attribute__((ext_vector_type(4)));
        const uint8_t *col = matrix + c0;
        u32x4 nx = *reinterpret_cast<const u32x4 *>(col + (uint64_t)order[0] * pitch);
        for (int s = 0; s < n; s++) {
            const u32x4 cur = nx;
            if (s + 1 < n) nx = *reinterpret_cast<const u32x4 *>(col + (uint64_t)order[s + 1] * pitch);
#pragma unroll
            for (int i = 0; i < 16; i++) {
                const uint32_t code = s_lut[(cur[i >> 2] >> (8 * (i & 3))) & 0xFFu];
                if (code == 0xFF) { bad |= 1u << i; continue; }
                if (code) { pu[i] += 1u + (((code & (code - 1)) == 0) ? 0x10000u : 0u); m[i] |= 1u << code; }
            }
        }
        uint32_t kw[4] = {0, 0, 0, 0};
#pragma unroll
        for (int i = 0; i < 16; i++) {
            const uint32_t present = pu[i] & 0xFFFFu, unambig = pu[i] >> 16, count = ambig_as_missing ? unambig : present;
            uint32_t k;
            if (present == 0) k = 2;
            else if (ambig_as_missing && count == 0) k = 2;
            else if ((uint64_t)count < min_count) k = 0;
            else k = filter_type_keep(filter_type, ignore_const_gaps, m[i], present < (uint32_t)n);
            if (c0 + i < n_cols) {
                n_absent += present == 0; n_silent += present != 0 && k == 2; n_removed += k == 0;
                kw[i >> 2] |= k << (8 * (i & 3));
            }
        }
        if (c0 + 16 <= n_cols) {
            *reinterpret_cast<u32x4 *>(keep + c0) = u32x4{kw[0], kw[1], kw[2], kw[3]};
            if (bad) *bad_byte = 1;
        } else {
            for (int i = 0; i < 16 && c0 + i < n_cols; i++) { keep[c0 + i] = (uint8_t)(kw[i >> 2] >> (8 * (i & 3))); if ((bad >> i) & 1u) *bad_byte = 1; }
        }
    }
    for (int d = 32; d; d >>= 1) { n_absent += __shfl_down(n_absent, d, 64); n_silent += __shfl_down(n_silent, d, 64); n_removed += __shfl_down(n_removed, d, 64); }
    if ((threadIdx.x & 63) == 0) { s_cnt[threadIdx.x >> 6][0] = n_absent; s_cnt[threadIdx.x >> 6][1] = n_silent; s_cnt[threadIdx.x >> 6][2] = n_removed; }
    __syncthreads();
    if (threadIdx.x < 3) {
        const uint32_t t = s_cnt[0][threadIdx.x] + s_cnt[1][threadIdx.x] + s_cnt[2][threadIdx.x] + s_cnt[3][threadIdx.x];
        if (t) atomicAdd(&counts[threadIdx.x], (unsigned long long)t);
    }
}
void launch_subset_verdicts(const uint8_t *matrix, uint64_t pitch, const int *order, int n, uint64_t n_cols, uint64_t min_count, int ambig_as_missing,
                            int filter_type, int ignore_const_gaps, uint8_t *keep, unsigned long long *counts, int *bad_byte, hipStream_t st)
{
    if (!n_cols || n <= 0) return;
    hipLaunchKernelGGL(subset_verdict_kernel, dim3((unsigned)((n_cols + 4095) / 4096)), dim3(256), 0, st, matrix, pitch, order, n, n_cols, min_count,
                       ambig_as_missing, filter_type, ignore_const_gaps, keep, counts, bad_byte);
}
template <typename T>
__global__ void compact_vec_kernel(const T *in, T *out, uint64_t n, const uint8_t *keep, const uint64_t *pos)
{
    for (uint64_t c = (uint64_t)blockIdx.x * blockDim.x + threadIdx.x; c < n; c += (uint64_t)gridDim.x * blockDim.x)
        if (keep[c] == 1) out[pos[c]] = in[c];
}
void launch_compact_u32(const uint32_t *in, uint32_t *out, uint64_t n, const uint8_t *keep, const uint64_t *pos, hipStream_t st)
{
    if (!n) return;
    uint64_t g = (n + 255) / 256; if (g > 8192) g = 8192;
    hipLaunchKernelGGL(compact_vec_kernel<uint32_t>, dim3((unsigned)g), dim3(256), 0, st, in, out, n, keep, pos);
}
void launch_compact_u64(const uint64_t *in, uint64_t *out, uint64_t n, const uint8_t *keep, const uint64_t *pos, hipStream_t st)
{
    if (!n) return;
    uint64_t g = (n + 255) / 256; if (g > 8192) g = 8192;
    hipLaunchKernelGGL(compact_vec_kernel<uint64_t>, dim3((unsigned)g), dim3(256), 0, st, in, out, n, keep, pos);
}
struct alignas(16) pair64 { uint64_t a, b; };
void launch_compact_u128(const uint64_t *in, uint64_t *out, uint64_t n, const uint8_t *keep, const uint64_t *pos, hipStream_t st)
{
    if (!n) return;
    uint64_t g = (n + 255) / 256; if (g > 8192) g = 8192;
    hipLaunchKernelGGL(compact_vec_kernel<pair64>, dim3((unsigned)g), dim3(256), 0, st, (const pair64 *)in, (pair64 *)out, n, keep, pos);
}
__global__ void mask_ambig_stats_kernel(uint32_t *mask, uint64_t n)
{
    const uint64_t c = (uint64_t)blockIdx.x * blockDim.x + threadIdx.x;
    if (c >= n) return;
    const uint32_t acgt = (1u << 1) | (1u << 2) | (1u << 4) | (1u << 8);
    uint32_t m = mask[c];
    if (m & ~acgt) m = (m & acgt) | (1u << 15);
    mask[c] = m;
}
void launch_mask_ambig_stats(uint32_t *mask, uint64_t n, hipStream_t st)
{
    if (!n) return;
    hipLaunchKernelGGL(mask_ambig_stats_kernel, dim3((unsigned)((n + 255) / 256)), dim3(256), 0, st, mask, n);
}

__global__ __launch_bounds__(256) void row_stats_rm_kernel(const uint8_t *cells, uint64_t S, uint64_t nr, uint32_t *present, uint32_t *unambig,
                                                           uint32_t *mask, int *bad_byte)
{
    __shared__ uint8_t s_lut[256];
    s_lut[threadIdx.x] = (uint8_t)set_code(threadIdx.x);
    __syncthreads();
    const int lane = threadIdx.x & 63;
    const uint64_t waves = (uint64_t)gridDim.x * 4;
    for (uint64_t r = (uint64_t)blockIdx.x * 4 + (threadIdx.x >> 6); r < nr; r += waves) {
        const int64_t b = (int64_t)(r * S), e = b + (int64_t)S;
        const int64_t skew = (int64_t)(((uintptr_t)cells + (uintptr_t)b) & 3u);
        uint32_t p = 0, u = 0, m = 0; bool bad = false;
        for (int64_t a = b - skew + 4 * lane; a < e; a += 256) {
            const uint32_t x = *reinterpret_cast<const uint32_t *>(cells + a);
#pragma unroll
            for (int i = 0; i < 4; i++) {
                const int64_t q = a + i;
                if (q < b || q >= e) continue;
                const uint32_t code = s_lut[(x >> (8 * i)) & 0xFFu];
                if (code == 0xFF) { bad = true; continue; }
                if (code) { p++; u += (code & (code - 1)) == 0; m |= 1u << code; }
            }
        }
        for (int d = 32; d; d >>= 1) { p += __shfl_down(p, d, 64); u += __shfl_down(u, d, 64); m |= __shfl_down(m, d, 64); }
        if (lane == 0) { present[r] = p; unambig[r] = u; mask[r] = m; }
        if (bad) *bad_byte = 1;
    }
}
void launch_row_stats_rm(const uint8_t *cells, uint64_t S, uint64_t nr, uint32_t *present, uint32_t *unambig, uint32_t *mask, int *bad_byte, hipStream_t st)
{
    if (!nr || !S) return;
    const uint64_t g = (nr + 3) / 4 < 65536 ? (nr + 3) / 4 : 65536;
    hipLaunchKernelGGL(row_stats_rm_kernel, dim3((unsigned)g), dim3(256), 0, st, cells, S, nr, present, unambig, mask, bad_byte);
}
constexpr int RM_ROWS = 512;
__global__ __launch_bounds__(256) void compact_rm_kernel(const uint8_t *cells, uint64_t S, uint64_t nr, const uint8_t *keep, const uint64_t *pos,
                                                         uint8_t *out, uint64_t pitch, uint64_t col0, int mask_ambig)
{
    __shared__ uint16_t s_rows[RM_ROWS];
    __shared__ uint32_t s_n;
    __shared__ uint8_t s_tile[64][RM_ROWS + 4];
    const uint64_t r0 = (uint64_t)blockIdx.x * RM_ROWS, c0 = (uint64_t)blockIdx.y * 64;
    const uint32_t rows_here = (uint32_t)(nr - r0 < (uint64_t)RM_ROWS ? nr - r0 : (uint64_t)RM_ROWS);
    if (threadIdx.x == 0) s_n = 0;
    __syncthreads();
    const uint64_t p0 = pos[r0];
    for (uint32_t i = threadIdx.x; i < rows_here; i += 256)
        if (keep[r0 + i] == 1) { s_rows[(uint32_t)(pos[r0 + i] - p0)] = (uint16_t)i; atomicAdd(&s_n, 1u); }
    __syncthreads();
    const uint32_t kn = s_n;
    if (!kn) return;
    const uint32_t cols_here = (uint32_t)(S - c0 < 64 ? S - c0 : 64);
    const int lane = threadIdx.x & 63, wv = threadIdx.x >> 6;
    for (uint32_t j = wv; j < kn; j += 4) {
// ... 619 lines not shown
```

ska.rust_amd/csrc/skx_internal.h:

```cpp
#pragma once
#include "../../include/skx.h"
#include "skx_device.h"
#include <atomic>
#include <chrono>
#include <cstdio>
#include <condition_variable>
#include <functional>
#include <memory>
#include <mutex>
#include <new>
#include <thread>
#include <sys/types.h>
#include <stdexcept>
#include <string>
#include <vector>

namespace skx {

void set_error(const char *fmt, ...);

int hip_fail(hipError_t e, const char *what);

#define SKX_HIP(call) do { hipError_t e_ = (call); if (e_ != hipSuccess) return skx::hip_fail(e_, #call); } while (0)
#define SKX_TRY(call) do { int r_ = (call); if (r_ != SKX_OK) return r_; } while (0)

void phase_add(const char *name, double secs);
struct PhaseTimer {
    const char *name; std::chrono::steady_clock::time_point t0;
    explicit PhaseTimer(const char *n) : name(n), t0(std::chrono::steady_clock::now()) {}
    double stop() { double s = 0; if (name) { s = std::chrono::duration<double>(std::chrono::steady_clock::now() - t0).count(); phase_add(name, s); name = nullptr; } return s; }
    ~PhaseTimer() { stop(); }
};

void *dev_alloc(size_t bytes, hipError_t *err);
void dev_free(void *p);
void dev_trim();

template <typename T>
struct DevBuf {
    T *p = nullptr; size_t n = 0;
    DevBuf() = default;
    DevBuf(const DevBuf &) = delete;
    DevBuf &operator=(const DevBuf &) = delete;
    DevBuf(DevBuf &&o) noexcept : p(o.p), n(o.n) { o.p = nullptr; o.n = 0; }
    DevBuf &operator=(DevBuf &&o) noexcept { if (this != &o) { release(); p = o.p; n = o.n; o.p = nullptr; o.n = 0; } return *this; }
    ~DevBuf() { release(); }
    void release() { if (p) dev_free(p); p = nullptr; n = 0; }
    int alloc(size_t count) {
        release();
        if (!count) count = 1;
        hipError_t e = hipSuccess;
        p = (T *)dev_alloc(count * sizeof(T), &e);
        if (!p) return hip_fail(e, "hipMalloc");
        n = count; return SKX_OK;
    }
    int zero(hipStream_t st) { return p ? (hipMemsetAsync(p, 0, n * sizeof(T), st) == hipSuccess ? SKX_OK : SKX_ENODEV) : SKX_OK; }
};

}

namespace skx {
struct Preallocator {
    int fd; off_t base;
    std::mutex mu; std::condition_variable cv; uint64_t target = 0, done = 0; bool stop = false;
    std::atomic<bool> failed{false};
    std::thread th;
    Preallocator(int fd_, off_t base_);
    ~Preallocator();
    void raise(uint64_t bytes);
    void finish(uint64_t bytes);
};
}

struct skx_ctx {
    int expect_fd = -1;
    int device = 0;
    hipStream_t stream = nullptr;
    hipEvent_t ev[4] = {nullptr, nullptr, nullptr, nullptr};
    skx_timings tm{};
    bool timing = true;
    std::string merge_path;
};

namespace skx {
struct StageTimer {
    skx_ctx *c; double *slot;
    StageTimer(skx_ctx *c_, double *s) : c(c_), slot(s) { if (c->timing) (void)hipEventRecord(c->ev[0], c->stream); }
    ~StageTimer()
    {
        if (!c->timing) return;
        (void)hipEventRecord(c->ev[1], c->stream);
        (void)hipEventSynchronize(c->ev[1]);
        float ms = 0; if (hipEventElapsedTime(&ms, c->ev[0], c->ev[1]) == hipSuccess) *slot += ms;
    }
};
uint64_t next_object_id();
}
struct skx_dictset {
    const uint64_t id = skx::next_object_id();
    skx_ctx *ctx = nullptr;
    int n = 0, k = 0, rc = 0, logB = 0, key_bits = 64;
    skx::HashParams hp{};
    skx::WideHash wh{};
    bool wide() const { return key_bits == 128; }
    skx::DevBuf<uint64_t> words;
    skx::DevBuf<uint64_t> off;
    skx::DevBuf<uint32_t> raw;
    skx::DevBuf<uint32_t> ucnt;
    skx::DevBuf<uint16_t> sidx;
    int sb = 0;
    std::vector<uint64_t> sample_size;
    bool sorted = true;
    uint32_t region_cap = 0; uint64_t maxlen = 0;
    std::vector<uint64_t> raw_total;
    skx::DictView view() const { return skx::DictView{words.p, off.p, ucnt.p, n, logB, wide() ? wh.bits : hp.bits, sidx.p, sb}; }
};

struct skx_pieces {
    skx::DevBuf<uint8_t> data;
    skx::DevBuf<uint16_t> plen;
    skx::DevBuf<uint16_t> perm;
    skx::DevBuf<uint32_t> nrank;
    uint32_t cap = 0; int logQ = 0;
    std::vector<uint64_t> sample_cells;
};

struct skx_keyset {
    skx_ctx *ctx = nullptr;
    int k = 0, rc = 0, logN = 0;
    skx::HashParams hp{};
    skx::WideHash wh{};
    bool wide = false;
    int wpk() const { return wide ? 2 : 1; }
    uint32_t stride = 0, max_rows = 0;
    uint64_t total = 0;
    skx::DevBuf<uint64_t> stage;
    skx::DevBuf<uint32_t> ncnt;
    skx::DevBuf<uint64_t> roff;
    skx::DevBuf<uint64_t> flat;
    std::vector<uint64_t> h_roff;
    skx::DevBuf<uint16_t> side;
    skx::DevBuf<uint16_t> perm;
    const skx_dictset *side_of = nullptr;
    skx::DevBuf<uint16_t> g_perm;
    skx::DevBuf<uint32_t> g_n;
    skx::DevBuf<uint64_t> g_base;
    int l_logN = -1; uint32_t l_stride = 0, g_max = 0;
    skx_pieces *pieces = nullptr; const skx_dictset *pieces_of = nullptr; uint64_t pieces_of_id = 0;
    bool holds_pieces_of(const skx_dictset *d) const { return pieces && pieces_of == d && d && pieces_of_id == d->id; }
    skx_keyset() = default;
    skx_keyset(const skx_keyset &) = delete; skx_keyset &operator=(const skx_keyset &) = delete;
    ~skx_keyset() { delete pieces; }
};

struct skx_array {
    skx_ctx *ctx = nullptr;
    int k = 0, rc = 0, k_bits = 64;
    skx::HashParams hp{};
    std::vector<std::string> names;
    std::string version;
    uint64_t n_kmers = 0;
    uint64_t n_rows = 0;
    uint64_t pitch = 0;
    uint64_t total_samples = 0;
// ... 199 lines not shown
```

ska.rust_amd/skx_engine.py:

```python
import ctypes as C
import os

import numpy as np

HERE = os.path.dirname(os.path.abspath(__file__))
LIB_PATH = os.path.join(HERE, "libskx.so")

QUAL_NOFILTER, QUAL_MIDDLE, QUAL_STRICT = 0, 1, 2
FILTER_NONE, FILTER_NO_CONST, FILTER_NO_AMBIG, FILTER_NO_AMBIG_OR_CONST = 0, 1, 2, 3
OK, EINVAL, EIO, ENODEV, ENOMEM, EEMPTY, EUNSUP, EFORMAT = range(8)

KEY_DT = np.dtype([("lo", "<u8"), ("hi", "<u8")])
DIST_DT = np.dtype([("distance", "<f8"), ("mismatch_prop", "<f8"), ("match_count", "<u8"), ("mismatch_count", "<u8")])
PAIR_DT = np.dtype([("i", "<u4"), ("j", "<u4"), ("d", DIST_DT)])
NJ_DT = np.dtype([("a", "<u4"), ("b", "<u4"), ("len_a", "<f8"), ("len_b", "<f8")])


class Qual(C.Structure):
    _fields_ = [("min_count", C.c_uint16), ("min_qual", C.c_uint8), ("qual_filter", C.c_int32)]


class Stream(C.Structure):
    _fields_ = [("seq", C.c_void_p), ("qual", C.c_void_p), ("len", C.c_uint64)]

# ... 4 lines not shown


class ArrayInfo(C.Structure):
    _fields_ = [("k", C.c_int32), ("rc", C.c_int32), ("k_bits", C.c_int32), ("n_kmers", C.c_uint64),
                ("n_rows", C.c_uint64), ("n_samples", C.c_uint64), ("total_samples", C.c_uint64)]


class Timings(C.Structure):
    _fields_ = [(n, C.c_double) for n in ("hist", "scatter", "dedupe", "key_union", "assemble", "filter", "compact", "distance",
                                                 "append_probe", "append", "pieces_stats", "pieces_rows")]


class Job(C.Structure):
    _fields_ = [("names", C.POINTER(C.c_char_p)), ("file1", C.POINTER(C.c_char_p)), ("file2", C.POINTER(C.c_char_p)), ("n_samples", C.c_int),
                ("k", C.c_int), ("rc", C.c_int), ("qual", Qual), ("threads", C.c_int), ("proportion_reads", C.c_double),
                ("output", C.c_char_p), ("merge_parts", C.c_int), ("min_freq", C.c_double),
                ("filter_type", C.c_int), ("mask_ambig", C.c_int), ("ignore_const_gaps", C.c_int), ("filter_ambig_as_missing", C.c_int),
                ("filt_ambig", C.c_int), ("extras", C.c_void_p)]


class DistExtras(C.Structure):
    _fields_ = [("tree", C.c_char_p), ("clusters", C.c_char_p), ("cluster_snps", C.c_double), ("cluster_mismatches", C.c_double)]


class SelectSpec(C.Structure):
    _fields_ = [("max_snps", C.c_double), ("max_mismatches", C.c_double), ("closest", C.c_int32), ("band_rows", C.c_int32)]

    @classmethod
    def of(cls, max_snps=None, max_mismatches=None, closest=0, band_rows=0):
        return cls(-1.0 if max_snps is None else float(max_snps), -1.0 if max_mismatches is None else float(max_mismatches), int(closest), int(band_rows))


class SelectInfo(C.Structure):
    _fields_ = [("bands", C.c_uint64), ("band_rows", C.c_uint64), ("count_buffer_bytes", C.c_uint64), ("candidates", C.c_uint64)]


class MstSpec(C.Structure):
    _fields_ = [("max_snps", C.c_double), ("max_mismatches", C.c_double), ("band_rows", C.c_int32)]

    @classmethod
    def of(cls, max_snps=None, max_mismatches=None, band_rows=0):
        return cls(-1.0 if max_snps is None else float(max_snps), -1.0 if max_mismatches is None else float(max_mismatches), int(band_rows))


class MstInfo(C.Structure):
    _fields_ = [(f, C.c_uint64) for f in ("bands", "band_rows", "count_buffer_bytes", "candidates", "edges", "components", "rounds")]


class BandedSpec(C.Structure):
    _fields_ = [("cluster_snps", C.c_double), ("cluster_mismatches", C.c_double), ("band_rows", C.c_int32)]


class BandedInfo(C.Structure):
    _fields_ = [("bands", C.c_uint64), ("band_rows", C.c_uint64), ("count_buffer_bytes", C.c_uint64), ("edges", C.c_uint64), ("clusters", C.c_uint64)]


class SubsetInfo(C.Structure):
    _fields_ = [("rows_present", C.c_uint64), ("removed", C.c_uint64), ("silent", C.c_uint64), ("sites", C.c_uint64)]


class EngineError(RuntimeError):
    def __init__(self, code, msg):
        super().__init__(f"[skx {code}] {msg}")
        self.code = code


SYMBOLS = """skx_last_error skx_version skx_ctx_create skx_ctx_destroy skx_ctx_sync skx_ctx_stream skx_dictset_build
skx_dictset_build_files skx_read_records skx_dictset_free skx_dictset_nsamples skx_dictset_key_bits skx_dictset_size skx_dictset_export
skx_keyset_union skx_keyset_union_notes skx_keyset_size skx_keyset_device skx_keyset_from_device skx_keyset_merge skx_keyset_free
skx_array_assemble skx_array_assemble_lazy skx_merge skx_build_and_merge skx_array_free skx_array_save skx_array_load skx_array_from_host
skx_array_info skx_array_name skx_array_version skx_array_export skx_array_sample_kmers skx_array_pieces_info skx_array_filter
skx_array_write_fasta skx_array_fasta skx_array_device_matrix skx_array_device_stats skx_array_set_total_samples skx_array_distance skx_free skx_ctx_timings skx_ctx_merge_path
skx_array_merge skx_array_delete_samples skx_array_weed skx_keyset_from_fasta skx_array_ctx skx_set_last_error skx_array_map skx_cov_histogram skx_phases_json skx_phase_add skx_skf_peek_k skx_array_load_filtered skx_ctx_expect_output skx_array_distance_planes skx_planes_distance skx_array_distance_filtered
skx_comm_unique_id skx_comm_create skx_comm_create_local skx_comm_destroy skx_comm_rank skx_comm_world skx_comm_bytes_received skx_comm_transport skx_comm_barrier
skx_comm_allgather skx_comm_allreduce_u32 skx_comm_gather_root skx_shard_range skx_pair_bands skx_keyset_allgather skx_array_reduce_stats skx_array_distance_sharded
skh_build_sharded skh_align_sharded skh_distance_sharded
skh_apply_filters skh_align skh_align_fd skh_distance_tsv skh_nk skh_save_skf skh_load_array skh_sample_name skh_main skh_merge skh_delete skh_weed skh_cov skh_cov_fit skh_align_inputs_fd skh_distance_skf_tsv skh_help skh_log
skx_array_lo_graph skx_lo_graph_info skx_lo_graph_export skx_lo_gather skx_lo_graph_free skh_lo
skx_dist_nj skx_matrix_nj skh_nj_newick skh_distance_clusters skh_distance_skf_tsv_extras
skx_array_distance_query skx_array_distance_query_filtered skh_distance_query_tsv
skx_array_distance_select skx_array_distance_select_prefiltered skh_distance_select_tsv
skx_array_distance_banded skx_array_distance_banded_prefiltered skh_clusters_csv skh_cluster_cutoffs skh_distance_banded_files
skx_array_subset_filtered skh_read_groups skh_align_groups skh_align_samples_fd
skx_array_distance_mst skx_array_distance_mst_prefiltered skh_distance_mst_tsv skh_mst_levels_csv""".split()

_lib = None


def load_library():
    global _lib
    if _lib is not None:
        return _lib
    if not os.path.exists(LIB_PATH):
        raise ImportError(f"{LIB_PATH} not built: run `python -c 'import __graft_entry__ as g; g.build()'` "
                          f"(make -C ska.rust_amd). There is no fallback path.")
    lib = C.CDLL(LIB_PATH)
    vp, cp, i, d, u64 = C.c_void_p, C.c_char_p, C.c_int, C.c_double, C.c_uint64
    pp = C.POINTER(vp)
    lib.skx_last_error.restype = cp
    lib.skx_version.restype = cp
    lib.skx_ctx_create.argtypes = [i, pp]
    lib.skx_array_lo_graph.argtypes = [vp, pp]
    lib.skx_lo_graph_info.argtypes = [vp, C.POINTER(LoInfo)]
    lib.skx_lo_graph_export.argtypes = [vp, vp, vp, vp, vp, vp]
    lib.skx_lo_gather.argtypes = [vp, vp, u64, vp, vp]
    lib.skx_lo_graph_free.argtypes = [vp]
    lib.skh_lo.argtypes = [vp, cp, cp, cp, C.c_float, C.c_size_t, C.c_size_t, i]
    lib.skx_dist_nj.argtypes = [vp, vp, i, vp]
    lib.skx_matrix_nj.argtypes = [vp, vp, i, vp]
    lib.skh_nj_newick.argtypes = [C.POINTER(cp), vp, i, pp, C.POINTER(u64)]
    lib.skh_distance_clusters.argtypes = [C.POINTER(cp), vp, i, d, d, pp, C.POINTER(u64), pp, C.POINTER(u64)]
    lib.skh_distance_skf_tsv_extras.argtypes = [vp, cp, d, i, C.POINTER(DistExtras), pp, C.POINTER(u64)]
    lib.skx_array_distance_query.argtypes = [vp, d, i, vp, i, vp]
    lib.skx_array_distance_query_filtered.argtypes = [vp, d, i, vp, i, vp, C.POINTER(C.c_int64), C.POINTER(u64)]
    lib.skh_distance_query_tsv.argtypes = [vp, cp, cp, C.POINTER(cp), i, d, i, pp, C.POINTER(u64)]
    lib.skx_array_distance_select.argtypes = [vp, d, i, C.POINTER(SelectSpec), pp, C.POINTER(u64), C.POINTER(C.c_int64), C.POINTER(u64), C.POINTER(SelectInfo)]
    lib.skx_array_distance_select_prefiltered.argtypes = [vp, C.c_int64, i, C.POINTER(SelectSpec), pp, C.POINTER(u64), C.POINTER(SelectInfo)]
    lib.skh_distance_select_tsv.argtypes = [vp, cp, d, i, C.POINTER(SelectSpec), pp, C.POINTER(u64)]
    lib.skx_array_distance_banded.argtypes = [vp, d, i, C.POINTER(BandedSpec), vp, vp, C.POINTER(C.c_int64), C.POINTER(u64), C.POINTER(BandedInfo)]
    lib.skx_array_distance_banded_prefiltered.argtypes = [vp, C.c_int64, i, C.POINTER(BandedSpec), vp, vp, C.POINTER(BandedInfo)]
    lib.skh_clusters_csv.argtypes = [C.POINTER(cp), vp, i, pp, C.POINTER(u64)]
    lib.skh_cluster_cutoffs.argtypes = [d, d, i, C.POINTER(u64), C.POINTER(d)]
    lib.skh_distance_banded_files.argtypes = [vp, cp, d, i, C.POINTER(DistExtras)]
    lib.skx_array_distance_mst.argtypes = [vp, d, i, C.POINTER(MstSpec), pp, C.POINTER(u64), C.POINTER(C.c_int64), C.POINTER(u64), C.POINTER(MstInfo)]
    lib.skx_array_distance_mst_prefiltered.argtypes = [vp, C.c_int64, i, C.POINTER(MstSpec), pp, C.POINTER(u64), C.POINTER(MstInfo)]
    lib.skh_distance_mst_tsv.argtypes = [vp, cp, d, i, C.POINTER(MstSpec), pp, C.POINTER(u64)]
    lib.skh_mst_levels_csv.argtypes = [C.POINTER(cp), vp, u64, i, vp, i, pp, C.POINTER(u64)]
    lib.skx_array_subset_filtered.argtypes = [vp, vp, i, C.POINTER(FilterSpec), pp, C.POINTER(SubsetInfo)]
    lib.skh_read_groups.argtypes = [cp, pp, C.POINTER(u64), C.POINTER(u64)]
    lib.skh_align_groups.argtypes = [vp, C.POINTER(cp), i, i, i, i, i, d, i, cp, i, cp]
    lib.skh_align_samples_fd.argtypes = [vp, C.POINTER(cp), i, i, i, i, i, d, i, C.POINTER(cp), i, i]
    lib.skx_ctx_destroy.argtypes = [vp]
    lib.skx_ctx_sync.argtypes = [vp]
    lib.skx_ctx_stream.argtypes = [vp]
    lib.skx_ctx_stream.restype = vp
    lib.skx_ctx_timings.argtypes = [vp, C.POINTER(Timings), i]
    lib.skx_ctx_merge_path.argtypes = [vp]
    lib.skx_ctx_merge_path.restype = C.c_char_p
    lib.skx_dictset_build.argtypes = [vp, C.POINTER(Stream), i, i, i, i, C.POINTER(Qual), pp]
    lib.skx_dictset_build_files.argtypes = [vp, C.POINTER(cp), C.POINTER(cp), i, i, i, C.POINTER(Qual), i, d, pp]
    lib.skx_dictset_free.argtypes = [vp]
    lib.skx_dictset_nsamples.argtypes = [vp]
    lib.skx_dictset_key_bits.argtypes = [vp]
    lib.skx_dictset_size.argtypes = [vp, i, C.POINTER(u64)]
    lib.skx_dictset_export.argtypes = [vp, i, vp, vp, u64]
    lib.skx_keyset_union.argtypes = [vp, vp, pp]
    lib.skx_keyset_union_notes.argtypes = [vp, vp, pp]
    lib.skx_keyset_size.argtypes = [vp, C.POINTER(u64)]
    lib.skx_keyset_device.argtypes = [vp, pp, C.POINTER(u64), C.POINTER(i)]
    lib.skx_keyset_from_device.argtypes = [vp, vp, u64, i, i, pp]
    lib.skx_keyset_merge.argtypes = [vp, pp, i, pp]
    lib.skx_keyset_free.argtypes = [vp]
    lib.skx_array_assemble.argtypes = [vp, vp, vp, C.POINTER(cp), pp]
    lib.skx_array_assemble_lazy.argtypes = [vp, vp, vp, C.POINTER(cp), pp]
    lib.skx_merge.argtypes = [vp, vp, C.POINTER(cp), pp]
    lib.skx_build_and_merge.argtypes = [vp, C.POINTER(cp), C.POINTER(cp), C.POINTER(cp), i, i, i, C.POINTER(Qual), i, d, pp]
    lib.skx_array_free.argtypes = [vp]
    lib.skx_array_save.argtypes = [vp, cp]
    lib.skx_array_load.argtypes = [vp, cp, i, pp]
    lib.skx_array_from_host.argtypes = [vp, i, i, C.POINTER(cp), i, vp, vp, vp, u64, cp, pp]
    lib.skx_array_info.argtypes = [vp, C.POINTER(ArrayInfo)]
    lib.skx_array_name.argtypes = [vp, u64]
    lib.skx_array_name.restype = cp
    lib.skx_array_version.argtypes = [vp]
    lib.skx_array_version.restype = cp
    lib.skx_array_export.argtypes = [vp, vp, vp, vp]
    lib.skx_array_sample_kmers.argtypes = [vp, vp]
    lib.skx_array_pieces_info.argtypes = [vp, C.POINTER(u64), C.POINTER(u64), C.POINTER(C.c_uint32)]
    lib.skx_array_filter.argtypes = [vp, u64, i, i, i, i, i, C.POINTER(C.c_int32)]
    lib.skx_array_write_fasta.argtypes = [vp, i]
    lib.skx_array_fasta.argtypes = [vp, pp, C.POINTER(u64)]
    lib.skx_array_device_matrix.argtypes = [vp, pp, C.POINTER(u64), C.POINTER(u64)]
    lib.skx_array_device_stats.argtypes = [vp, pp, pp, pp, pp]
    lib.skx_array_set_total_samples.argtypes = [vp, u64]
    lib.skx_array_distance.argtypes = [vp, d, i, vp]
    lib.skx_free.argtypes = [vp]
    lib.skh_apply_filters.argtypes = [vp, d, i, i, i, i, C.POINTER(C.c_int32)]
    lib.skh_align.argtypes = [vp, i, i, i, d, i, pp, C.POINTER(u64)]
    lib.skh_distance_tsv.argtypes = [vp, d, i, pp, C.POINTER(u64)]
    lib.skh_nk.argtypes = [vp, i, pp, C.POINTER(u64)]
    lib.skh_save_skf.argtypes = [vp, cp]
    lib.skh_load_array.argtypes = [vp, C.POINTER(cp), i, i, pp]
    lib.skx_array_merge.argtypes = [vp, pp, i, pp]
    lib.skx_array_delete_samples.argtypes = [vp, C.POINTER(cp), i]
    lib.skx_array_weed.argtypes = [vp, vp, i, C.POINTER(u64)]
    lib.skx_keyset_from_fasta.argtypes = [vp, cp, i, i, pp]
    lib.skx_array_map.argtypes = [vp, cp, i, i, i, i, pp, C.POINTER(u64)]
    lib.skx_cov_histogram.argtypes = [vp, cp, cp, i, i, vp]
    lib.skh_cov.argtypes = [vp, cp, cp, i, i, pp, C.POINTER(u64), C.POINTER(u64)]
    lib.skh_cov_fit.argtypes = [vp, u64, C.POINTER(d), C.POINTER(d), C.POINTER(u64)]
    lib.skx_array_ctx.argtypes = [vp]
    lib.skx_array_ctx.restype = vp
    lib.skx_set_last_error.argtypes = [cp]
    lib.skh_merge.argtypes = [vp, C.POINTER(cp), i, cp]
    lib.skh_delete.argtypes = [vp, C.POINTER(cp), i, cp]
    lib.skh_weed.argtypes = [vp, cp, i, d, i, i, i, i, cp]
    lib.skx_read_records.argtypes = [cp, cp, d, i, pp, pp, C.POINTER(u64)]
    lib.skh_sample_name.argtypes = [cp]
    lib.skh_sample_name.restype = vp
    lib.skx_ctx_expect_output.argtypes = [vp, i]
    lib.skx_array_distance_planes.argtypes = [vp, i, pp, C.POINTER(u64), C.POINTER(i)]
    lib.skx_planes_distance.argtypes = [vp, vp, i, u64, i, d, i, i, vp]
    lib.skx_array_distance_filtered.argtypes = [vp, d, i, vp, C.POINTER(C.c_int64), C.POINTER(u64)]
    lib.skx_array_load_filtered.argtypes = [vp, cp, C.POINTER(FilterSpec), pp, C.POINTER(C.c_int64), C.POINTER(C.c_int64)]
    lib.skh_align_inputs_fd.argtypes = [vp, C.POINTER(cp), i, i, i, i, i, d, i, i]
    lib.skh_distance_skf_tsv.argtypes = [vp, cp, d, i, pp, C.POINTER(u64)]
    lib.skx_phases_json.argtypes = [pp, C.POINTER(u64), i]
    lib.skx_phase_add.argtypes = [cp, d]
    lib.skx_phase_add.restype = None
    lib.skx_comm_unique_id.argtypes = [vp]
    lib.skx_comm_create.argtypes = [vp, i, i, vp, pp]
    lib.skx_comm_create_local.argtypes = [vp, i, i, cp, pp]
    lib.skx_comm_destroy.argtypes = [vp]
    lib.skx_comm_destroy.restype = None
    lib.skx_comm_rank.argtypes = [vp]
    lib.skx_comm_world.argtypes = [vp]
    lib.skx_comm_bytes_received.argtypes = [vp]
    lib.skx_comm_bytes_received.restype = u64
    lib.skx_comm_transport.argtypes = [vp, C.POINTER(i), C.POINTER(i), C.POINTER(i)]
    lib.skx_comm_barrier.argtypes = [vp]
    lib.skx_comm_allgather.argtypes = [vp, vp, vp, u64, i]
# ... 86 lines not shown
    p = lib.skh_sample_name(path.encode())
    s = C.string_at(p).decode()
    lib.skx_free(p)
    return s


class LoInfo(C.Structure):
    _fields_ = [("k", C.c_int32), ("words_per_node", C.c_int32), ("n_samples", C.c_uint64), ("colour_words", C.c_uint64),
                ("n_nodes", C.c_uint64), ("n_edges", C.c_uint64), ("n_entries", C.c_uint64), ("n_colours", C.c_uint64), ("n_kmers", C.c_uint64)]


def _to_ints(words, wpn):
    if wpn == 1:
        return [int(x) for x in words]
    return [int(words[2 * i]) | (int(words[2 * i + 1]) << 64) for i in range(len(words) // 2)]


class LoGraph:

    def __init__(self, h):
        self.h = h
        inf = LoInfo()
        _check(_lib.skx_lo_graph_info(h, C.byref(inf)))
        self.info = {n: getattr(inf, n) for n, _ in LoInfo._fields_}
        w, N, E, X = inf.words_per_node, inf.n_nodes, inf.n_edges, inf.n_entries
        self.wpn = w
        self.nodes = np.zeros(N * w, np.uint64)
        self.offsets = np.zeros(N + 1, np.uint64)
        self.neighbours = np.zeros(E * w, np.uint64)
        self.entries = np.zeros(X * w, np.uint64)
        self.exits = np.zeros(X * w, np.uint64)
        _check(_lib.skx_lo_graph_export(h, self.nodes.ctypes.data, self.offsets.ctypes.data, self.neighbours.ctypes.data,
                                        self.entries.ctypes.data, self.exits.ctypes.data))

    def adjacency(self):
        nodes, nb = _to_ints(self.nodes, self.wpn), _to_ints(self.neighbours, self.wpn)
        off = [int(x) for x in self.offsets]
        return {n: nb[off[i]:off[i + 1]] for i, n in enumerate(nodes)}

    def gather(self, kmers):
        n, w = len(kmers), self.wpn
        q = np.zeros(max(1, n * w), np.uint64)
        for i, x in enumerate(kmers):
            for j in range(w):
                q[i * w + j] = (x >> (64 * j)) & 0xFFFFFFFFFFFFFFFF
        W = self.info["colour_words"]
        out = np.zeros(max(1, n * W), np.uint64)
        found = np.zeros(max(1, n), np.uint8)
        _check(_lib.skx_lo_gather(self.h, q.ctypes.data, n, out.ctypes.data, found.ctypes.data))
        cols = [sum(int(out[i * W + t]) << (64 * t) for t in range(W)) for i in range(n)]
        return cols, [bool(found[i]) for i in range(n)]

    def close(self):
        if getattr(self, "h", None) and _lib is not None:
            _lib.skx_lo_graph_free(self.h)
            self.h = None

    def __del__(self):
        self.close()


class Context:
    def __init__(self, device=0):
        lib = load_library()
        h = C.c_void_p()
        _check(lib.skx_ctx_create(device, C.byref(h)))
        self.h = h

    def sync(self):
        _check(_lib.skx_ctx_sync(self.h))

    @property
    def stream(self):
        return _lib.skx_ctx_stream(self.h)

    def timings(self, reset=False):
        t = Timings()
        _lib.skx_ctx_timings(self.h, C.byref(t), int(reset))
        return {n: getattr(t, n) for n, _ in Timings._fields_}

    def merge_path(self):
        return _lib.skx_ctx_merge_path(self.h).decode()

    def lo_graph(self, array):
        h = C.c_void_p()
        _check(_lib.skx_array_lo_graph(array.h, C.byref(h)))
        return LoGraph(h)

    def dist_nj(self, dist, n_samples):
        dist = np.ascontiguousarray(dist, DIST_DT)
        if n_samples >= 2 and dist.size != n_samples * (n_samples - 1) // 2:
            raise ValueError("the table does not hold n(n-1)/2 pairs")
        joins = np.zeros(max(n_samples - 1, 1), NJ_DT)
        _check(_lib.skx_dist_nj(self.h, _np_ptr(dist), n_samples, _np_ptr(joins)))
        return joins[: n_samples - 1]

    def matrix_nj(self, matrix):
        m = np.ascontiguousarray(matrix, np.float64)
        if m.ndim != 2 or m.shape[0] != m.shape[1]:
            raise ValueError("a square matrix is required")
        n = m.shape[0]
        joins = np.zeros(max(n - 1, 1), NJ_DT)
        _check(_lib.skx_matrix_nj(self.h, _np_ptr(m), n, _np_ptr(joins)))
        return joins[: n - 1]

    def distance_skf_tsv(self, skf_file, min_freq=0.0, filt_ambig=True, tree=None, clusters=None, cluster_snps=10.0, cluster_mismatches=1.0):
        x = DistExtras(tree.encode() if tree else None, clusters.encode() if clusters else None, cluster_snps, cluster_mismatches)
        p, n = C.c_void_p(), C.c_uint64()
        _check(_lib.skh_distance_skf_tsv_extras(self.h, skf_file.encode(), min_freq, int(filt_ambig), C.byref(x) if tree or clusters else None,
                                                C.byref(p), C.byref(n)))
        return _take(p, n)

    def distance_query_tsv(self, skf_file, names=(), query_skf=None, min_freq=0.0, filt_ambig=True):
        names = list(names)
        arr = (C.c_char_p * max(len(names), 1))(*[n.encode() for n in names])
        p, n = C.c_void_p(), C.c_uint64()
        _check(_lib.skh_distance_query_tsv(self.h, skf_file.encode(), query_skf.encode() if query_skf else None, arr, len(names), float(min_freq),
                                           int(filt_ambig), C.byref(p), C.byref(n)))
        return _take(p, n)

    def distance_select_tsv(self, skf_file, min_freq=0.0, filt_ambig=True, max_snps=None, max_mismatches=None, closest=0, band_rows=0):
        spec = SelectSpec.of(max_snps, max_mismatches, closest, band_rows)
        p, n = C.c_void_p(), C.c_uint64()
        _check(_lib.skh_distance_select_tsv(self.h, skf_file.encode(), float(min_freq), int(filt_ambig), C.byref(spec), C.byref(p), C.byref(n)))
        return _take(p, n)

    def distance_mst_tsv(self, skf_file, min_freq=0.0, filt_ambig=True, max_snps=None, max_mismatches=None, band_rows=0):
        spec = MstSpec.of(max_snps, max_mismatches, band_rows)
        p, n = C.c_void_p(), C.c_uint64()
        _check(_lib.skh_distance_mst_tsv(self.h, skf_file.encode(), float(min_freq), int(filt_ambig), C.byref(spec), C.byref(p), C.byref(n)))
        return _take(p, n)

    def distance_banded_files(self, skf_file, min_freq=0.0, filt_ambig=True, tree=None, clusters=None, cluster_snps=10.0, cluster_mismatches=1.0):
        x = DistExtras(tree.encode() if tree else None, clusters.encode() if clusters else None, cluster_snps, cluster_mismatches)
        _check(_lib.skh_distance_banded_files(self.h, skf_file.encode(), float(min_freq), int(filt_ambig), C.byref(x)))

    def align_groups(self, inputs, groups_file, out_prefix, min_group_size=2, threads=1, min_freq=0.9, filter_ambig_as_missing=False,
                     filter_type=FILTER_NO_CONST, mask_ambig=False, ignore_const_gaps=False):
        inputs = [inputs] if isinstance(inputs, str) else list(inputs)
        arr = (C.c_char_p * len(inputs))(*[x.encode() for x in inputs])
        _check(_lib.skh_align_groups(self.h, arr, len(inputs), int(threads), int(filter_type), int(mask_ambig), int(ignore_const_gaps), float(min_freq),
                                     int(filter_ambig_as_missing), groups_file.encode(), int(min_group_size), out_prefix.encode()))

    def align_samples(self, inputs, names, fd, threads=1, min_freq=0.9, filter_ambig_as_missing=False, filter_type=FILTER_NO_CONST, mask_ambig=False,
                      ignore_const_gaps=False):
        inputs = [inputs] if isinstance(inputs, str) else list(inputs)
        names = list(names)
        arr = (C.c_char_p * len(inputs))(*[x.encode() for x in inputs])
        nm = (C.c_char_p * max(len(names), 1))(*[x.encode() for x in names])
        _check(_lib.skh_align_samples_fd(self.h, arr, len(inputs), int(threads), int(filter_type), int(mask_ambig), int(ignore_const_gaps), float(min_freq),
                                         int(filter_ambig_as_missing), nm, len(names), int(fd)))

    def close(self):
        if getattr(self, "h", None) and _lib is not None:
            _lib.skx_ctx_destroy(self.h)
            self.h = None

    def __del__(self):
        self.close()


_default_ctx = None


def default_context():
    global _default_ctx
# ... 636 lines not shown
```

Baseline: 29410.

## Defer pieces stats to filter and bound read ranks by min_count cut

Pieces-based arrays no longer compute per-row stats eagerly at assembly. When filtering with min_count >= 2, a new per-block histogram kernel over piece lengths finds a rank cutoff beyond which no row can reach min_count. The stats kernel then skips those ranks and whole waves with no work. The rows kernel shrinks its per-sample read span to the highest kept rank, and four compaction launches are fused into one. This adds a kernel and some state-tracking complexity, and it is only exact if the rank-ordering assumption behind the cut holds.

```diff
diff --git a/include/skx.h b/include/skx.h
--- a/include/skx.h
+++ b/include/skx.h
@@ -202,6 +202,7 @@
 typedef struct { double hist, scatter, dedupe, key_union, assemble, filter, compact, distance, append_probe, append, pieces_stats, pieces_rows; } skx_timings;
 int  skx_ctx_timings(skx_ctx *ctx, skx_timings *t, int reset);
 const char *skx_ctx_merge_path(skx_ctx *ctx);
+int  skx_ctx_filter_cut(skx_ctx *ctx, uint64_t *ranks, uint64_t *blocks);
 
 #ifdef __cplusplus
 }
diff --git a/ska.rust_amd/csrc/skx_api.cpp b/ska.rust_amd/csrc/skx_api.cpp
--- a/ska.rust_amd/csrc/skx_api.cpp
+++ b/ska.rust_amd/csrc/skx_api.cpp
@@ -235,6 +235,30 @@
 extern "C" void *skx_ctx_stream(skx_ctx *c) { return (void *)c->stream; }
 uint64_t skx::next_object_id() { static std::atomic<uint64_t> n{0}; return ++n; }
 extern "C" const char *skx_ctx_merge_path(skx_ctx *c) { return c ? c->merge_path.c_str() : ""; }
+extern "C" int skx_ctx_filter_cut(skx_ctx *c, uint64_t *ranks, uint64_t *blocks)
+{
+    if (!c) { set_error("bad arguments"); return SKX_EINVAL; }
+    if (ranks) *ranks = c->cut_ranks;
+    if (blocks) *blocks = c->cut_blocks;
+    return SKX_OK;
+}
+extern "C" int skx_debug_pieces_cut(skx_ctx *ctx, const uint16_t *plen, int n_samples, int n_blocks, uint32_t cap, uint32_t min_count, uint32_t *out)
+{
+    return skx_guarded([&]() -> int {
+    if (!ctx || !plen || !out || n_samples < 1 || n_samples > 65535 || n_blocks < 1 || cap < 32u || cap % 32u || cap > 12032u) { set_error("bad arguments"); return SKX_EINVAL; }
+    SKX_HIP(hipSetDevice(ctx->device));
+    hipStream_t st = ctx->stream;
+    const uint64_t n = (uint64_t)n_blocks * (uint64_t)n_samples;
+    DevBuf<uint16_t> d_pl; DevBuf<uint32_t> d_cut;
+    SKX_TRY(d_pl.alloc(n)); SKX_TRY(d_cut.alloc((size_t)n_blocks));
+    SKX_HIP(hipMemcpyAsync(d_pl.p, plen, n * 2, hipMemcpyHostToDevice, st));
+    launch_pieces_cut(d_pl.p, n_samples, cap, min_count, nullptr, nullptr, 0, n_blocks, d_cut.p, nullptr, st);
+    SKX_HIP(hipMemcpyAsync(out, d_cut.p, (size_t)n_blocks * 4, hipMemcpyDeviceToHost, st));
+    SKX_HIP(hipStreamSynchronize(st));
+    SKX_HIP(hipGetLastError());
+    return SKX_OK;
+    });
+}
 extern "C" int skx_ctx_timings(skx_ctx *c, skx_timings *t, int reset)
 {
     return skx_guarded([&]() -> int {
@@ -1147,11 +1171,41 @@
     return array_make_lazy(ctx, d, rows, names, out);
     });
 }
+static int pieces_stats_pass(skx_array *a, uint64_t min_count)
+{
+    skx_ctx *ctx = a->ctx; hipStream_t st = ctx->stream;
+    const skx_pieces *pc = a->pieces; const skx_keyset *blk = a->lazy_rows;
+    const int S = (int)a->names.size(), nb = 1 << pc->logQ;
+    ctx->cut_ranks = ctx->cut_blocks = 0;
+    if (!a->n_rows) return SKX_OK;
+    const uint32_t stage = min_count >= 2 ? pieces_stats_bound(pc->cap) : 0u;
+    DevBuf<uint32_t> r_cut; DevBuf<unsigned long long> tally;
+    if (stage) { SKX_TRY(r_cut.alloc((size_t)nb)); SKX_TRY(tally.alloc(2)); SKX_TRY(tally.zero(st)); }
+    unsigned long long h_tally[2] = {0, 0};
+    {
+        StageTimer t(ctx, &ctx->tm.assemble);
+        KernelTimer kt(ctx, &ctx->tm.pieces_stats);
+        if (stage) launch_pieces_cut(pc->plen.p, S, pc->cap, (uint32_t)std::min<uint64_t>(min_count, 0xFFFFFFFEull), pc->nrank.p, blk->ncnt.p, stage, nb, r_cut.p, tally.p, st);
+        launch_pieces_stats(pc->data.p, pc->plen.p, pc->perm.p, pc->nrank.p, blk->ncnt.p, blk->roff.p, pc->cap, S, nb, a->present.p, a->unambig.p, a->mask.p, a->vcount.p, st,
+                            stage ? r_cut.p : nullptr);
+        if (stage) SKX_HIP(hipMemcpyAsync(h_tally, tally.p, 16, hipMemcpyDeviceToHost, st));
+    }
+    SKX_HIP(hipStreamSynchronize(st));
+    SKX_HIP(hipGetLastError());
+    ctx->cut_ranks = h_tally[0]; ctx->cut_blocks = h_tally[1];
+    if (stage && getenv("SKX_DEBUG")) fprintf(stderr, "[skx] filter: min_count %llu, the rank bound left %llu ranks unread over %llu of %d row blocks\n", (unsigned long long)min_count, h_tally[0], h_tally[1], nb);
+    return SKX_OK;
+}
 int skx::array_lazy_stats(skx_array *a)
 {
     if (!a->lazy() || a->stats_ready) return SKX_OK;
     skx_ctx *ctx = a->ctx; hipStream_t st = ctx->stream;
     SKX_HIP(hipSetDevice(ctx->device));
+    if (a->pieces) {
+        SKX_TRY(pieces_stats_pass(a, 0));
+        a->stats_ready = true;
+        return SKX_OK;
+    }
     DevBuf<int> d_flag; SKX_TRY(d_flag.alloc(1)); SKX_TRY(d_flag.zero(st));
     if (a->n_rows) {
         AssembleArgs aa = lazy_args(a, d_flag.p);
@@ -1167,6 +1221,7 @@
     if (!a->lazy()) return SKX_OK;
     skx_ctx *ctx = a->ctx; hipStream_t st = ctx->stream;
     SKX_HIP(hipSetDevice(ctx->device));
+    if (a->pieces) SKX_TRY(array_lazy_stats(a));
     const uint64_t U = a->n_rows; const size_t S = a->names.size();
     a->pitch = pitch_for(U);
     SKX_TRY(a->matrix.alloc((uint64_t)S * a->pitch));
@@ -1363,6 +1418,9 @@
         if (src->wide) launch_gather_keys_wide((const u128 *)src->stage.p, src->stride, g ? g->ncnt.p : blk->ncnt.p, g ? g->roff.p : blk->roff.p, 1 << src->logN, (u128 *)a->keys.p, st);
         else launch_gather_keys(src->stage.p, src->stride, g ? g->ncnt.p : blk->ncnt.p, g ? g->roff.p : blk->roff.p, 1 << src->logN, a->keys.p, 0, src->hp, st);
         if (g) { SKX_TRY(a->present.zero(st)); SKX_TRY(a->unambig.zero(st)); SKX_TRY(a->mask.zero(st)); SKX_TRY(a->vcount.zero(st)); }
+    }
+    if (!g && !knob("stats_eager")) a->stats_ready = false;
+    else if (U) {
         StageTimer t(ctx, &ctx->tm.assemble);
         KernelTimer kt(ctx, &ctx->tm.pieces_stats);
         launch_pieces_stats(pc->data.p, pc->plen.p, pc->perm.p, pc->nrank.p, blk->ncnt.p, blk->roff.p, pc->cap, S, 1 << logQ, a->present.p, a->unambig.p, a->mask.p, a->vcount.p, st);
@@ -1697,6 +1755,7 @@
     const uint64_t U = a->n_rows; const size_t S = a->names.size();
     const bool filter_ambig_as_missing = vcount_from_unambig;
     if (kept == U && !mask_ambig) {
+        a->stats_ready = true;
         if (filter_ambig_as_missing && U) SKX_HIP(hipMemcpyAsync(a->vcount.p, a->unambig.p, U * 4, hipMemcpyDeviceToDevice, st));
         SKX_HIP(hipStreamSynchronize(st));
         return SKX_OK;
@@ -1708,7 +1767,7 @@
         SKX_TRY(nm.alloc((uint64_t)S * np)); SKX_TRY(p2.alloc(kept)); SKX_TRY(u2.alloc(kept)); SKX_TRY(m2.alloc(kept)); SKX_TRY(v2.alloc(kept));
         if (a->pieces) {
             PiecesRowsArgs pa = pieces_args(a);
-            pa.out = nm.p; pa.pitch = np; pa.keep = keep.p; pa.kpos = pos.p; pa.mask_ambig = mask_ambig;
+            pa.out = nm.p; pa.pitch = np; pa.keep = keep.p; pa.kpos = pos.p; pa.mask_ambig = mask_ambig; pa.full_pieces = knob("stats_eager") ? 1 : 0;
             KernelTimer kt(ctx, &ctx->tm.pieces_rows);
             launch_pieces_rows(pa, 1u << a->pieces->logQ, st);
         } else if (a->lazy()) {
@@ -1719,10 +1778,11 @@
             SKX_TRY(lazy_check_missing(a, d_flag));
         } else
             launch_compact_matrix(a->matrix.p, a->pitch, nm.p, np, (int)S, U, keep.p, pos.p, mask_ambig, st);
-        launch_compact_u32(a->present.p, p2.p, U, keep.p, pos.p, st);
-        launch_compact_u32(a->unambig.p, u2.p, U, keep.p, pos.p, st);
-        launch_compact_u32(a->mask.p, m2.p, U, keep.p, pos.p, st);
-        launch_compact_u32(filter_ambig_as_missing ? a->unambig.p : a->vcount.p, v2.p, U, keep.p, pos.p, st);
+        {
+            const uint32_t *const in[4] = {a->present.p, a->unambig.p, a->mask.p, filter_ambig_as_missing ? a->unambig.p : a->vcount.p};
+            uint32_t *const out[4] = {p2.p, u2.p, m2.p, v2.p};
+            launch_compact_stats(in, out, U, keep.p, pos.p, st);
+        }
         if (mask_ambig) launch_mask_ambig_stats(m2.p, kept, st);
         if (a->n_kmers == U && keys_follow) {
             if (a->k <= 31) {
@@ -1747,6 +1807,7 @@
         a->matrix = std::move(nm); a->present = std::move(p2); a->unambig = std::move(u2); a->mask = std::move(m2); a->vcount = std::move(v2);
         a->pitch = np; a->n_rows = kept;
         a->drop_lazy();
+        a->stats_ready = true;
     }
     return SKX_OK;
 }
@@ -1758,7 +1819,11 @@
     skx_ctx *ctx = a->ctx; hipStream_t st = ctx->stream;
     SKX_HIP(hipSetDevice(ctx->device));
     const uint64_t U = a->n_rows; const size_t S = a->names.size();
-    SKX_TRY(array_lazy_stats(a));
+    ctx->cut_ranks = ctx->cut_blocks = 0;
+    if (a->pieces && !a->stats_ready && !filter_ambig_as_missing && min_count >= 2 && a->total_samples == 0 && !knob("stats_eager"))
+        SKX_TRY(pieces_stats_pass(a, min_count));
+    else
+        SKX_TRY(array_lazy_stats(a));
     DevBuf<uint8_t> keep; DevBuf<uint64_t> pos;
     SKX_TRY(keep.alloc(U)); SKX_TRY(pos.alloc(U + 1));
     uint64_t kept = 0, silent = 0;
diff --git a/ska.rust_amd/csrc/skx_append.hip b/ska.rust_amd/csrc/skx_append.hip
--- a/ska.rust_amd/csrc/skx_append.hip
+++ b/ska.rust_amd/csrc/skx_append.hip
@@ -482,9 +482,53 @@
 void launch_append(const AppendArgs &a, uint32_t region_cap, hipStream_t st) { (void)region_cap; launch_append_t<false>(a, (1u << a.logQ) / a.rounds, st); }
 void launch_append_probe(const AppendArgs &a, uint32_t region_cap, unsigned blocks, hipStream_t st) { (void)region_cap; launch_append_t<true>(a, blocks, st); }
 
+__global__ __launch_bounds__(256) void pieces_cut_kernel(const uint16_t *plen, int S, uint32_t cap, uint32_t min_count, const uint32_t *nrank, const uint32_t *ncnt,
+                                                         uint32_t stage, uint32_t *r_cut, unsigned long long *tally)
+{
+    extern __shared__ uint32_t s_hist[];
+    __shared__ uint32_t s_sum[256];
+    __shared__ uint32_t s_cut;
+    const uint64_t j = blockIdx.x;
+    const uint32_t tid = threadIdx.x, nbin = cap + 1u, share = (nbin + 255u) / 256u;
+    for (uint32_t i = tid; i < nbin; i += 256) s_hist[i] = 0;
+    if (tid == 0) s_cut = 0;
+    __syncthreads();
+    const uint16_t *pl = plen + j * (uint64_t)S;
+    for (int s = (int)tid; s < S; s += 256) { const uint32_t v = pl[s]; atomicAdd(&s_hist[v < cap ? v : cap], 1u); }
+    __syncthreads();
+    const uint32_t b0 = tid * share, b1 = b0 + share < nbin ? b0 + share : nbin;
+    uint32_t own = 0;
+    for (uint32_t b = b0; b < b1; b++) own += s_hist[b];
+    s_sum[tid] = own;
+    __syncthreads();
+    uint32_t above = 0;
+    for (uint32_t t = tid + 1; t < 256; t++) above += s_sum[t];
+    if (min_count >= 1u && above < min_count && min_count <= above + own) {
+        uint32_t acc = above;
+        for (uint32_t b = b1; b-- > b0;) { acc += s_hist[b]; if (acc >= min_count) { s_cut = b; break; } }
+    }
+    __syncthreads();
+    if (tid == 0) {
+        uint32_t rc = min_count ? s_cut : 0xFFFFFFFFu;
+        if (ncnt && ncnt[j] > stage) rc = 0xFFFFFFFFu;
+        r_cut[j] = rc;
+        if (tally && nrank) {
+            const uint32_t nr = nrank[j], lim = nr < rc ? nr : rc;
+            const uint64_t seen = (uint64_t)((lim + 31u) / 32u) * 32u;
+            if (seen < nr) { atomicAdd(&tally[0], (unsigned long long)(nr - seen)); atomicAdd(&tally[1], 1ull); }
+        }
+    }
+}
+void launch_pieces_cut(const uint16_t *plen, int n_samples, uint32_t cap, uint32_t min_count, const uint32_t *nrank, const uint32_t *ncnt, uint32_t stage, int n_blocks,
+                       uint32_t *r_cut, unsigned long long *tally, hipStream_t st)
+{
+    if (n_blocks <= 0) return;
+    hipLaunchKernelGGL(pieces_cut_kernel, dim3((unsigned)n_blocks), dim3(256), ((size_t)cap + 1) * 4, st, plen, n_samples, cap, min_count, nrank, ncnt, stage, r_cut, tally);
+}
+
 __global__ __launch_bounds__(256) void pieces_stats_kernel(const uint8_t *pieces, const uint16_t *plen, const uint16_t *perm, const uint32_t *nrank, const uint32_t *ncnt,
                                                            const uint64_t *roff, uint32_t cap, int S, uint32_t *o_present, uint32_t *o_unambig, uint32_t *o_mask,
-                                                           uint32_t *o_vcount, int force_direct, uint32_t stage)
+                                                           uint32_t *o_vcount, int force_direct, uint32_t stage, const uint32_t *r_cut)
 {
     constexpr int W = 4;
     extern __shared__ __attribute__((aligned(16))) uint16_t s_stage[];
@@ -504,7 +548,11 @@
     const uint16_t *pl = plen + j * (uint64_t)S;
     const uint4 *col = reinterpret_cast<const uint4 *>(pieces + j * (uint64_t)S * (cap / 2)) + d;
     const uint32_t step = cap / 32;
-    const bool mine = d * 32u < nr;
+    uint32_t lim = nr;
+    if (r_cut && staged) { const uint32_t rc = r_cut[j]; if (rc < lim) lim = rc; }
+    const uint32_t nseen = (lim + 31u) / 32u * 32u < nr ? (lim + 31u) / 32u * 32u : nr;
+    const bool mine = d * 32u < lim;
+    const bool wave_has = (d - (uint32_t)(threadIdx.x & 63)) * 32u < lim;
     uint32_t pN[W], aN[W];
     uint32_t pE[W], pO[W], aE[W], aO[W], uni[W];
     uint32_t PE0[W], PE1[W], PO0[W], PO1[W], AE0[W], AE1[W], AO0[W], AO1[W];
@@ -535,7 +583,7 @@
         pN[w] += nz; aN[w] += am;
         uni[w] |= x;
     };
-    for (int s0 = 0, since = 0, nib = 0; s0 < S; s0 += 64) {
+    for (int s0 = 0, since = 0, nib = 0; wave_has && s0 < S; s0 += 64) {
         const uint32_t plv = s0 + lane < S ? (uint32_t)pl[s0 + lane] : 0u;
         const int n = S - s0 < 64 ? S - s0 : 64;
 #pragma unroll 1
@@ -587,7 +635,7 @@
     }
     if (!staged) __threadfence();
     __syncthreads();
-    const uint32_t rk0 = blockIdx.y * 256u * 8u * W, rk1 = rk0 + 256u * 8u * W < nr ? rk0 + 256u * 8u * W : nr;
+    const uint32_t rk0 = blockIdx.y * 256u * 8u * W, rk1 = rk0 + 256u * 8u * W < nseen ? rk0 + 256u * 8u * W : nseen;
     for (uint32_t rb = rk0 + (uint32_t)wv * 64u; rb < rk1; rb += 256u) {
         const uint32_t rr = rb + (uint32_t)lane;
         uint32_t pp = 0xFFFFu; bool hit = false;
@@ -623,16 +671,24 @@
         o_unambig[r0 + p] = s_un[p]; o_mask[r0 + p] = s_mk[p];
     }
 }
+namespace {
+struct StatsLaunch { unsigned gy; int direct; uint32_t stage; bool bounded() const { return gy == 1 && !direct; } };
+StatsLaunch stats_launch(uint32_t cap)
+{
+    static const int direct = knob("stats_direct") ? 1 : 0;
+    return {(cap / 32 + 255u) / 256u, direct, (cap + 63u) / 64u * 64u};
+}
+}
 void launch_pieces_stats(const uint8_t *pieces, const uint16_t *plen, const uint16_t *perm, const uint32_t *nrank, const uint32_t *ncnt, const uint64_t *roff, uint32_t cap,
-                         int n_samples, int n_blocks, uint32_t *present, uint32_t *unambig, uint32_t *mask, uint32_t *vcount, hipStream_t st)
+                         int n_samples, int n_blocks, uint32_t *present, uint32_t *unambig, uint32_t *mask, uint32_t *vcount, hipStream_t st, const uint32_t *r_cut)
 {
     if (n_blocks <= 0) return;
-    const unsigned gy = (cap / 32 + 255u) / 256u;
-    static const int direct = knob("stats_direct") ? 1 : 0;
-    const uint32_t stage = (cap + 63u) / 64u * 64u;
-    hipLaunchKernelGGL(pieces_stats_kernel, dim3((unsigned)n_blocks, gy), dim3(256), (size_t)stage * 6, st, pieces, plen, perm, nrank, ncnt, roff, cap, n_samples, present, unambig, mask, vcount,
-                       direct, stage);
-}
+    const StatsLaunch l = stats_launch(cap);
+    if (!l.bounded()) r_cut = nullptr;
+    hipLaunchKernelGGL(pieces_stats_kernel, dim3((unsigned)n_blocks, l.gy), dim3(256), (size_t)l.stage * 6, st, pieces, plen, perm, nrank, ncnt, roff, cap, n_samples, present, unambig, mask, vcount,
+                       l.direct, l.stage, r_cut);
+}
+uint32_t pieces_stats_bound(uint32_t cap) { const StatsLaunch l = stats_launch(cap); return l.bounded() ? l.stage : 0u; }
 __global__ __launch_bounds__(256) void pieces_cells_kernel(const uint8_t *pieces, const uint16_t *plen, uint32_t cap, int S, unsigned long long *out)
 {
     const uint64_t j = blockIdx.x;
@@ -702,11 +758,14 @@
     const int s_lo = blockIdx.y * a.samples_per_wg, s_hi = s_lo + a.samples_per_wg < S ? s_lo + a.samples_per_wg : S;
     uint32_t *pc = s_piece + (size_t)wv * (cap / 8 + 4);
     const unsigned char *pcb = reinterpret_cast<const unsigned char *>(pc);
-    const uint32_t nrw = (nr + 7u) / 8u;
+    __shared__ uint32_t s_top;
+    uint32_t nrw = (nr + 7u) / 8u;
     if (lane < 4) pc[cap / 8 + lane] = 0u;
     for (uint32_t t0 = 0; t0 < nout + shift; t0 += cap) {
         for (uint32_t i = tid; i < cap + 16u; i += blockDim.x) s_src[i] = (uint16_t)cap;
+        if (KEPT && tid == 0) s_top = 0;
         __syncthreads();
+        uint32_t top = 0;
         for (uint32_t r = tid; r < nr; r += blockDim.x) {
             const uint32_t p = pj[r];
             if (p == 0xFFFFu || p >= n) continue;
@@ -714,9 +773,11 @@
             if (!KEPT) sc = shift + p;
             else if (a.keep[r0 + p] == 1) sc = shift + (uint32_t)(a.kpos[r0 + p] - k0);
             else continue;
-            if (sc >= t0 && sc < t0 + cap) s_src[sc - t0] = (uint16_t)r;
-        }
+            if (sc >= t0 && sc < t0 + cap) { s_src[sc - t0] = (uint16_t)r; top = r + 1u; }
+        }
+        if (KEPT && top) atomicMax(&s_top, top);
         __syncthreads();
+        if (KEPT && !a.full_pieces) nrw = (s_top + 7u) / 8u;
         const uint32_t v_lo = t0 / 4u, v_hi = (t0 + cap) / 4u < ndw ? (t0 + cap) / 4u : ndw;
         for (int s = s_lo + wv; s < s_hi; s += PR_WAVES) {
             const uint32_t pl = a.plen[j * (uint64_t)S + s];
diff --git a/ska.rust_amd/csrc/skx_device.h b/ska.rust_amd/csrc/skx_device.h
--- a/ska.rust_amd/csrc/skx_device.h
+++ b/ska.rust_amd/csrc/skx_device.h
@@ -150,7 +150,10 @@
 void launch_append_wide(const AppendArgs &a, hipStream_t st);
 void launch_append_wide_probe(const AppendArgs &a, unsigned blocks, hipStream_t st);
 void launch_pieces_stats(const uint8_t *pieces, const uint16_t *plen, const uint16_t *perm, const uint32_t *nrank, const uint32_t *ncnt, const uint64_t *roff, uint32_t cap,
-                         int n_samples, int n_blocks, uint32_t *present, uint32_t *unambig, uint32_t *mask, uint32_t *vcount, hipStream_t st);
+                         int n_samples, int n_blocks, uint32_t *present, uint32_t *unambig, uint32_t *mask, uint32_t *vcount, hipStream_t st, const uint32_t *r_cut = nullptr);
+void launch_pieces_cut(const uint16_t *plen, int n_samples, uint32_t cap, uint32_t min_count, const uint32_t *nrank, const uint32_t *ncnt, uint32_t stage, int n_blocks,
+                       uint32_t *r_cut, unsigned long long *tally, hipStream_t st);
+uint32_t pieces_stats_bound(uint32_t cap);
 void launch_pieces_cells(const uint8_t *pieces, const uint16_t *plen, uint32_t cap, int n_samples, int n_blocks, unsigned long long *out, hipStream_t st);
 void launch_region_totals(const uint32_t *raw, int n_samples, int logB, unsigned long long *out, hipStream_t st);
 struct PiecesRowsArgs {
@@ -160,6 +163,7 @@
     uint32_t j_base = 0; uint64_t col_base = 0;
     const uint8_t *keep = nullptr; const uint64_t *kpos = nullptr;
     int mask_ambig = 0;
+    int full_pieces = 0;
     int samples_per_wg = 0;
 };
 void launch_pieces_rows(const PiecesRowsArgs &a, uint32_t n_blocks, hipStream_t st);
@@ -189,6 +193,7 @@
 void launch_subset_verdicts(const uint8_t *matrix, uint64_t pitch, const int *order, int n, uint64_t n_cols, uint64_t min_count, int ambig_as_missing,
                             int filter_type, int ignore_const_gaps, uint8_t *keep, unsigned long long *counts, int *bad_byte, hipStream_t st);
 void launch_compact_u32(const uint32_t *in, uint32_t *out, uint64_t n, const uint8_t *keep, const uint64_t *pos, hipStream_t st);
+void launch_compact_stats(const uint32_t *const in[4], uint32_t *const out[4], uint64_t n, const uint8_t *keep, const uint64_t *pos, hipStream_t st);
 void launch_compact_u64(const uint64_t *in, uint64_t *out, uint64_t n, const uint8_t *keep, const uint64_t *pos, hipStream_t st);
 void launch_compact_u128(const uint64_t *in, uint64_t *out, uint64_t n, const uint8_t *keep, const uint64_t *pos, hipStream_t st);
 void launch_mask_ambig_stats(uint32_t *mask, uint64_t n, hipStream_t st);
diff --git a/ska.rust_amd/csrc/skx_device2.inc b/ska.rust_amd/csrc/skx_device2.inc
--- a/ska.rust_amd/csrc/skx_device2.inc
+++ b/ska.rust_amd/csrc/skx_device2.inc
@@ -219,6 +219,24 @@
     if (!n) return;
     uint64_t g = (n + 255) / 256; if (g > 8192) g = 8192;
     hipLaunchKernelGGL(compact_vec_kernel<uint32_t>, dim3((unsigned)g), dim3(256), 0, st, in, out, n, keep, pos);
+}
+struct CompactStats { const uint32_t *in[4]; uint32_t *out[4]; };
+__global__ void compact_stats_kernel(CompactStats a, uint64_t n, const uint8_t *keep, const uint64_t *pos)
+{
+    for (uint64_t c = (uint64_t)blockIdx.x * blockDim.x + threadIdx.x; c < n; c += (uint64_t)gridDim.x * blockDim.x)
+        if (keep[c] == 1) {
+            const uint64_t o = pos[c];
+#pragma unroll
+            for (int i = 0; i < 4; i++) a.out[i][o] = a.in[i][c];
+        }
+}
+void launch_compact_stats(const uint32_t *const in[4], uint32_t *const out[4], uint64_t n, const uint8_t *keep, const uint64_t *pos, hipStream_t st)
+{
+    if (!n) return;
+    CompactStats a;
+    for (int i = 0; i < 4; i++) { a.in[i] = in[i]; a.out[i] = out[i]; }
+    uint64_t g = (n + 255) / 256; if (g > 8192) g = 8192;
+    hipLaunchKernelGGL(compact_stats_kernel, dim3((unsigned)g), dim3(256), 0, st, a, n, keep, pos);
 }
 void launch_compact_u64(const uint64_t *in, uint64_t *out, uint64_t n, const uint8_t *keep, const uint64_t *pos, hipStream_t st)
 {
diff --git a/ska.rust_amd/csrc/skx_internal.h b/ska.rust_amd/csrc/skx_internal.h
--- a/ska.rust_amd/csrc/skx_internal.h
+++ b/ska.rust_amd/csrc/skx_internal.h
@@ -80,6 +80,7 @@
     skx_timings tm{};
     bool timing = true;
     std::string merge_path;
+    uint64_t cut_ranks = 0, cut_blocks = 0;
 };
 
 namespace skx {
diff --git a/ska.rust_amd/skx_engine.py b/ska.rust_amd/skx_engine.py
--- a/ska.rust_amd/skx_engine.py
+++ b/ska.rust_amd/skx_engine.py
@@ -110,7 +110,8 @@
 skx_array_distance_select skx_array_distance_select_prefiltered skh_distance_select_tsv
 skx_array_distance_banded skx_array_distance_banded_prefiltered skh_clusters_csv skh_cluster_cutoffs skh_distance_banded_files
 skx_array_subset_filtered skh_read_groups skh_align_groups skh_align_samples_fd
-skx_array_distance_mst skx_array_distance_mst_prefiltered skh_distance_mst_tsv skh_mst_levels_csv""".split()
+skx_array_distance_mst skx_array_distance_mst_prefiltered skh_distance_mst_tsv skh_mst_levels_csv
+skx_ctx_filter_cut""".split()
 
 _lib = None
 
@@ -165,6 +166,7 @@
     lib.skx_ctx_timings.argtypes = [vp, C.POINTER(Timings), i]
     lib.skx_ctx_merge_path.argtypes = [vp]
     lib.skx_ctx_merge_path.restype = C.c_char_p
+    lib.skx_ctx_filter_cut.argtypes = [vp, C.POINTER(u64), C.POINTER(u64)]
     lib.skx_dictset_build.argtypes = [vp, C.POINTER(Stream), i, i, i, i, C.POINTER(Qual), pp]
     lib.skx_dictset_build_files.argtypes = [vp, C.POINTER(cp), C.POINTER(cp), i, i, i, C.POINTER(Qual), i, d, pp]
     lib.skx_dictset_free.argtypes = [vp]
@@ -417,6 +419,11 @@
     def merge_path(self):
         return _lib.skx_ctx_merge_path(self.h).decode()
 
+    def filter_cut(self):
+        r, b = C.c_uint64(0), C.c_uint64(0)
+        _check(_lib.skx_ctx_filter_cut(self.h, C.byref(r), C.byref(b)))
+        return int(r.value), int(b.value)
+
     def lo_graph(self, array):
         h = C.c_void_p()
         _check(_lib.skx_array_lo_graph(array.h, C.byref(h)))
```

Result: faster. 29940 (median of 6 runs) (+1.8%).
